# Anannayjain/SNN_Object_DetectionDDP

Measured on NVIDIA B200. Metric: train images/sec, higher is better.
Workload: dtype bf16

## Files before the change

### include/snn_b200.h

```cpp
#ifndef SNN_B200_H
#define SNN_B200_H
#include <stdint.h>
#ifdef __cplusplus
extern "C" {
#endif

const char* snn_last_error(void);
int snn_version(void);
void snn_debug_set(int key, int value);
void snn_set_tile_scheduling(int dynamic);
int snn_conv_plan(int kind, int geom, int NB, int H, int W, int Cin, int Cout, int out_f32, int frames_per_step, int accumulate,
                  int* out20);
void snn_set_deterministic(int on);
int snn_get_deterministic(void);
void snn_set_dependent_launch(int on);
int snn_get_dependent_launch(void);
void snn_tensor_map_cache_stats(unsigned long long* hits, unsigned long long* misses);

enum { SNN_GEOM_3x3_S1 = 0, SNN_GEOM_3x3_S2 = 1, SNN_GEOM_1x1 = 2, SNN_GEOM_T2x2_S2 = 3 };
enum { SNN_ACT_LIF = 0, SNN_ACT_SILU = 1 };

int snn_conv_fprop(int geom, int NB, int H, int W,
                   const void* x0, int C0, long long ld0, const void* x1, int C1, long long ld1,
                   const void* w_bf16, int w_rows, int w_K, int w_coff, int Cout, int w_row_off,
                   const float* bias, void* out, int out_is_f32, long long out_ld, int out_coff,
                   int accumulate, void* stream);
long long snn_conv_stats_groups(int geom, int NB, int H, int W, int frames_per_step, int* groups_per_step);
int snn_conv_fprop_stats(int geom, int NB, int H, int W,
                         const void* x0, int C0, long long ld0, const void* x1, int C1, long long ld1,
                         const void* w_bf16, int w_rows, int w_K, int w_coff, int Cout, int w_row_off,
                         float* out, int frames_per_step, float* partials, void* stream);
int snn_bn_stats_from_partials(const float* partials, double* sums , int T, int C, int groups_per_step,
                               void* stream);
long long snn_bn_finalize_workspace_doubles(int T, int C, int groups_per_step);
int snn_bn_finalize_partials(const float* partials, double* sums, double* workspace, const float* gamma, const float* beta,
                             float* running_mean, float* running_var, long long* num_batches_tracked,
                             float* scale, float* shift, float* mean, float* invstd ,
                             unsigned int* counters, int T, int C, int P, int groups_per_step, float eps, float momentum,
                             void* stream);
int snn_conv_dgrad(int geom, int NB, int H, int W,
                   const void* dy, int Cout, long long ld_dy,
                   const void* w_bf16 , int w_K, int ci_off, int Ci,
                   void* dx, int dx_is_f32, long long dx_ld, int dx_coff, int accumulate, void* stream);
int snn_conv_wgrad(int geom, int NB, int H, int W,
                   const void* x, int Ci, long long ld_x, const void* dy, int Cout, long long ld_dy,
                   float* dw, int w_K, int w_coff, void* stream);
int snn_weight_prep(const float* w, void* w_bf16, void* wt_bf16, int N, int T, int K, void* stream);

long long snn_bn_stats_workspace_floats(int T, int P, int C);
int snn_bn_stats(const float* y, double* sums , float* workspace, int T, int P, int C, void* stream);
int snn_bn_finalize(const double* sums, const float* gamma, const float* beta,
                    float* running_mean, float* running_var,
                    float* scale, float* shift, float* mean, float* invstd ,
                    int T, int C, int P, float eps, float momentum, int training, void* stream);
int snn_bn_act_fwd(int act, const float* y, const float* scale, const float* shift, const float* v_init,
                   void* out_bf16, uint8_t* mask, float* v_final, int T, long long n_per_t, int C,
                   int ss_stride_t, float beta, float theta, void* stream);
int snn_bn_act_bwd(int act, int training, const float* y, const float* scale, const float* shift,
                   const float* mean, const float* invstd, const float* v_init,
                   const void* gs_bf16, const float* gv_final,
                   float* gx, void* dy_bf16, float* gv_init, float* red,
                   int T, int P, int C, int ss_stride_t, float beta, float theta, float alpha, void* stream);
int snn_bn_act_bwd2(int pass, int act, const float* y, const float* scale, const float* shift, const float* mean,
                    const float* invstd, const float* beta_bn, const float* v_init, const void* gs_bf16,
                    const float* gv_final, float* red, void* dy_bf16, float* gv_init, float* dgamma, float* dbeta,
                    int T, int P, int C, float beta, float theta, float alpha, void* stream);
int snn_bn_bwd_dx(const float* red, const float* gamma, const float* gx, const float* y,
                  const float* scale, const float* mean, const float* invstd, float* coef ,
                  float* dgamma, float* dbeta, void* dy_bf16, int T, int P, int C, void* stream);

int snn_lstm_gates_fwd(const float* gates, const float* c_prev, float* c_next, float* h_next,
                       void* h_bf16, long long P, int Ch, void* stream);
int snn_lstm_gates_bwd(const float* gates, const float* c_prev, const float* c_next,
                       const float* dh, const void* dh_bf16, const float* dc_in, void* dgates_bf16, float* dc_prev,
                       long long P, int Ch, void* stream);

int snn_nchw_to_nhwc(const float* in, void* out, int out_is_bf16, int NB, int C, int HW,
                     long long out_ld, int out_coff, void* stream);
int snn_nhwc_to_nchw(const void* in, int in_is_bf16, float* out, int NB, int C, int HW,
                     long long in_ld, int in_coff, void* stream);

int snn_dw3x3_fprop(const void* x_bf16, const float* w, float* y, int NB, int H, int W, int C, void* stream);
int snn_dw3x3_dgrad(const void* dy_bf16, const float* w, void* dx_bf16, int NB, int H, int W, int C, void* stream);
int snn_dw3x3_wgrad(const void* x_bf16, const void* dy_bf16, float* dw, int NB, int H, int W, int C, void* stream);
long long snn_dw3x3_stats_blocks(int frames_per_step, int W, int C);
int snn_dw3x3_fprop_stats(const void* x_bf16, const float* w9c, float* y, int NB, int H, int W, int C, int T, float* partials,
                          void* stream);

int snn_space_to_depth8(const float* frames, void* out_bf16, int B, int T, int H, int W, void* stream);
int snn_space_to_depth8_u8(const unsigned char* frames, void* out_bf16, int B, int T, int H, int W, void* stream);

int snn_bilinear_resize(int backward, const void* src_bf16, void* dst_bf16, int NB, int Hi, int Wi, int Ho, int Wo, int C,
                        void* stream);
int snn_nhwc_pad_crop(const void* src_bf16, void* dst_bf16, int NB, int Hs, int Ws, int Hd, int Wd, int C, void* stream);

int snn_colsum_bf16(const void* dy_bf16, float* acc, long long P, int C, void* stream);

int snn_grad_sumsq(const float* g, long long n, double* acc, int zero_first, void* stream);
int snn_adamw_step(float* p, float* g, float* m, float* v, void* shadow_bf16, long long n,
                   const float* hp, const double* sumsq, float* gnorm_out, int* step_ptr, int n_rows, int zero_grad,
                   void* stream);

int snn_detect_decode(const float* distri, const float* scores, const float* anchors, const float* stride,
                      int B, int A, int nc, int reg_max, int xywh, float* boxes, float* probs, void* stream);

long long snn_nms_workspace_keys(int nc, int A, int multi_label);
int snn_nms(const float* pred, int B, int nc, int A, float conf_thres, float iou_thres, int multi_label, int agnostic,
            int max_det, int max_nms, float max_wh, unsigned long long* keys, long long keys_per_image,
            float* out, int* out_idx, int* counts, void* stream);

int snn_det_match(const float* rows, const int* counts, int B, int max_det, const long long* gt_cls, const float* gt_box,
                  const unsigned char* gt_valid, int M, float img_w, float img_h, const float* iou_thres, int nc,
                  float* rec_conf, int* rec_cls, unsigned short* rec_tp, long long* rec_key, long long capacity,
                  long long* cursor, unsigned int* ticket, long long* n_gt, int* err, void* stream);
int snn_det_metrics_finalize(const long long* keys, const long long* order, const unsigned short* rec_tp, long long n,
                             const long long* n_gt, int nc, const int* err, double* curves, double* out, void* stream);

int snn_detect_loss_fwd(const float* distri, const float* scores, const float* anchors, const float* stride,
                        const float* tbox_px, const float* tscores, const uint8_t* fg, int B, int A, int nc, int reg_max,
                        double* sums, void* stream);
int snn_detect_loss_bwd(const float* distri, const float* scores, const float* anchors, const float* stride,
                        const float* tbox_px, const float* tscores, const uint8_t* fg, int B, int A, int nc, int reg_max,
                        const float* coef, float* g_distri, float* g_scores, void* stream);

long long snn_tal_workspace_bytes(int B, int A, int M);
int snn_detect_assign_loss_fwd(const float* distri, const float* scores, int nl, const int* a_off, const float* anchors,
                               const float* stride, const long long* gt_cls, const float* gt_box, const unsigned char* gt_valid,
                               float img_w, float img_h, int B, int A, int M, int nc, int reg_max, int topk, const float* gains,
                               void* workspace, float* pboxes, float* probs, float* tbox_px, float* tscores, unsigned char* fg,
                               double* sums, unsigned int* counter, float* out6, float* coef3, void* stream);
int snn_tal_assign(const float* probs, const float* pboxes, const float* anchors, const float* stride, const long long* gt_cls,
                   const float* gt_box, const unsigned char* gt_valid, float img_w, float img_h, int B, int A, int M, int nc, int topk,
                   void* workspace, float* tbox_px, float* tscores, unsigned char* fg, void* stream);
int snn_detect_loss_bwd_rows(const float* distri, const float* scores, int nl, const int* a_off, const float* anchors,
                             const float* stride, const float* tbox_px, const float* tscores, const unsigned char* fg, int B, int A,
                             int nc, int reg_max, const float* coef3, const float* gout3, void* g_distri, void* g_scores,
                             int out_is_bf16, void* stream);

#ifdef __cplusplus
}
#endif
#endif
```

### snn_object_detectionddp_b200/_lib.py

```python
import ctypes
import os

import torch

_HERE = os.path.dirname(os.path.abspath(__file__))
LIB_PATH = os.path.join(_HERE, "libsnnb200.so")

GEOM_3x3_S1, GEOM_3x3_S2, GEOM_1x1, GEOM_T2x2_S2 = 0, 1, 2, 3
ACT_LIF, ACT_SILU = 0, 1
GEOM_TAPS = {GEOM_3x3_S1: 9, GEOM_3x3_S2: 9, GEOM_1x1: 1, GEOM_T2x2_S2: 4}

_c = ctypes
_P, _I, _L, _F = _c.c_void_p, _c.c_int, _c.c_longlong, _c.c_float

_SIGNATURES = {
    "snn_conv_fprop": [_I, _I, _I, _I, _P, _I, _L, _P, _I, _L, _P, _I, _I, _I, _I, _I, _P, _P, _I, _L, _I, _I, _P],
    "snn_conv_fprop_stats": [_I, _I, _I, _I, _P, _I, _L, _P, _I, _L, _P, _I, _I, _I, _I, _I, _P, _I, _P, _P],
    "snn_bn_stats_from_partials": [_P, _P, _I, _I, _I, _P],
    "snn_bn_finalize_partials": [_P, _P, _P, _P, _P, _P, _P, _P, _P, _P, _P, _P, _P, _I, _I, _I, _I, _F, _F, _P],
    "snn_conv_dgrad": [_I, _I, _I, _I, _P, _I, _L, _P, _I, _I, _I, _P, _I, _L, _I, _I, _P],
    "snn_conv_wgrad": [_I, _I, _I, _I, _P, _I, _L, _P, _I, _L, _P, _I, _I, _P],
    "snn_weight_prep": [_P, _P, _P, _I, _I, _I, _P],
    "snn_bn_stats": [_P, _P, _P, _I, _I, _I, _P],
    "snn_bn_finalize": [_P, _P, _P, _P, _P, _P, _P, _P, _P, _I, _I, _I, _F, _F, _I, _P],
    "snn_bn_act_fwd": [_I, _P, _P, _P, _P, _P, _P, _P, _I, _L, _I, _I, _F, _F, _P],
    "snn_bn_act_bwd": [_I, _I, _P, _P, _P, _P, _P, _P, _P, _P, _P, _P, _P, _P, _I, _I, _I, _I, _F, _F, _F, _P],
    "snn_bn_act_bwd2": [_I, _I, _P, _P, _P, _P, _P, _P, _P, _P, _P, _P, _P, _P, _P, _P, _I, _I, _I, _F, _F, _F, _P],
    "snn_bn_bwd_dx": [_P, _P, _P, _P, _P, _P, _P, _P, _P, _P, _P, _I, _I, _I, _P],
    "snn_lstm_gates_fwd": [_P, _P, _P, _P, _P, _L, _I, _P],
    "snn_lstm_gates_bwd": [_P, _P, _P, _P, _P, _P, _P, _P, _L, _I, _P],
    "snn_nchw_to_nhwc": [_P, _P, _I, _I, _I, _I, _L, _I, _P],
    "snn_nhwc_to_nchw": [_P, _I, _P, _I, _I, _I, _L, _I, _P],
    "snn_colsum_bf16": [_P, _P, _L, _I, _P],
    "snn_bilinear_resize": [_I, _P, _P, _I, _I, _I, _I, _I, _I, _P],
    "snn_nhwc_pad_crop": [_P, _P, _I, _I, _I, _I, _I, _I, _P],
    "snn_dw3x3_fprop": [_P, _P, _P, _I, _I, _I, _I, _P],
    "snn_dw3x3_fprop_stats": [_P, _P, _P, _I, _I, _I, _I, _I, _P, _P],
    "snn_dw3x3_dgrad": [_P, _P, _P, _I, _I, _I, _I, _P],
    "snn_dw3x3_wgrad": [_P, _P, _P, _I, _I, _I, _I, _P],
    "snn_space_to_depth8": [_P, _P, _I, _I, _I, _I, _P],
    "snn_space_to_depth8_u8": [_P, _P, _I, _I, _I, _I, _P],
    "snn_detect_decode": [_P, _P, _P, _P, _I, _I, _I, _I, _I, _P, _P, _P],
    "snn_detect_loss_fwd": [_P, _P, _P, _P, _P, _P, _P, _I, _I, _I, _I, _P, _P],
    "snn_detect_loss_bwd": [_P, _P, _P, _P, _P, _P, _P, _I, _I, _I, _I, _P, _P, _P, _P],
    "snn_detect_assign_loss_fwd": [_P, _P, _I, _P, _P, _P, _P, _P, _P, _F, _F, _I, _I, _I, _I, _I, _I, _P, _P, _P, _P, _P, _P, _P, _P,
                                   _P, _P, _P, _P],
    "snn_tal_assign": [_P, _P, _P, _P, _P, _P, _P, _F, _F, _I, _I, _I, _I, _I, _P, _P, _P, _P, _P],
    "snn_detect_loss_bwd_rows": [_P, _P, _I, _P, _P, _P, _P, _P, _P, _I, _I, _I, _I, _P, _P, _P, _P, _I, _P],
    "snn_nms": [_P, _I, _I, _I, _F, _F, _I, _I, _I, _I, _F, _P, _L, _P, _P, _P, _P],
    "snn_det_match": [_P, _P, _I, _I, _P, _P, _P, _I, _F, _F, _P, _I, _P, _P, _P, _P, _L, _P, _P, _P, _P, _P],
    "snn_det_metrics_finalize": [_P, _P, _P, _L, _P, _I, _P, _P, _P, _P],
    "snn_grad_sumsq": [_P, _L, _P, _I, _P],
    "snn_adamw_step": [_P, _P, _P, _P, _P, _L, _P, _P, _P, _P, _I, _I, _P],
}

_lib = None
launch_count = 0


class SnnKernelError(RuntimeError):
    pass


def exported_symbols():
    return sorted(list(_SIGNATURES) + ["snn_last_error", "snn_version", "snn_debug_set", "snn_set_tile_scheduling", "snn_set_dependent_launch", "snn_get_dependent_launch", "snn_set_deterministic", "snn_get_deterministic", "snn_conv_plan", "snn_tensor_map_cache_stats", "snn_conv_stats_groups", "snn_bn_stats_workspace_floats", "snn_nms_workspace_keys",
                                             "snn_tal_workspace_bytes", "snn_dw3x3_stats_blocks", "snn_bn_finalize_workspace_doubles"])


def lib():
    global _lib
    if _lib is None:
        if not os.path.isfile(LIB_PATH):
            raise SnnKernelError(
                f"{LIB_PATH} not found: build it with `python -c 'import __graft_entry__ as g; g.build()'` "
                "(nvcc, sm_100a). There is no fallback path.")
        L = ctypes.CDLL(LIB_PATH)
        for name, args in _SIGNATURES.items():
            fn = getattr(L, name)
            fn.argtypes = args
            fn.restype = _I
        L.snn_last_error.restype = ctypes.c_char_p
        L.snn_version.restype = _I
        L.snn_conv_stats_groups.argtypes = [_I, _I, _I, _I, _I, ctypes.POINTER(_I)]
        L.snn_conv_stats_groups.restype = _L
        L.snn_bn_stats_workspace_floats.argtypes = [_I, _I, _I]
        L.snn_bn_stats_workspace_floats.restype = _L
        L.snn_nms_workspace_keys.argtypes = [_I, _I, _I]
        L.snn_nms_workspace_keys.restype = _L
        L.snn_bn_finalize_workspace_doubles.argtypes = [_I, _I, _I]
        L.snn_bn_finalize_workspace_doubles.restype = _L
        L.snn_dw3x3_stats_blocks.argtypes = [_I, _I, _I]
        L.snn_dw3x3_stats_blocks.restype = _L
        L.snn_tal_workspace_bytes.argtypes = [_I, _I, _I]
        L.snn_tal_workspace_bytes.restype = _L
        L.snn_debug_set.argtypes = [_I, _I]
        L.snn_debug_set.restype = None
        if "SNN_WGRAD_STRIP" in os.environ:
            L.snn_debug_set(13, int(os.environ["SNN_WGRAD_STRIP"]))
        if "SNN_WGRAD_ROUNDS" in os.environ:
            L.snn_debug_set(14, int(os.environ["SNN_WGRAD_ROUNDS"]))
        if "SNN_ROW_STRIP" in os.environ:
            L.snn_debug_set(12, int(os.environ["SNN_ROW_STRIP"]))
        L.snn_set_tile_scheduling.argtypes = [_I]
        L.snn_set_tile_scheduling.restype = None
        L.snn_set_dependent_launch.argtypes = [_I]
        L.snn_set_dependent_launch.restype = None
        L.snn_get_dependent_launch.argtypes = []
        L.snn_get_dependent_launch.restype = _I
        L.snn_set_dependent_launch(int(os.environ.get("SNN_DEPENDENT_LAUNCH", "0")))
        L.snn_conv_plan.argtypes = [_I] * 10 + [ctypes.POINTER(_I)]
        L.snn_conv_plan.restype = _I
        L.snn_set_deterministic.argtypes = [_I]
        L.snn_set_deterministic.restype = None
        L.snn_get_deterministic.argtypes = []
        L.snn_get_deterministic.restype = _I
        L.snn_set_deterministic(int(os.environ.get("SNN_DETERMINISTIC", "0")))
        L.snn_tensor_map_cache_stats.argtypes = [ctypes.POINTER(ctypes.c_ulonglong), ctypes.POINTER(ctypes.c_ulonglong)]
        L.snn_tensor_map_cache_stats.restype = None
        _lib = L
    return _lib


def ptr(t):
    if t is None:
        return None
    return t.data_ptr()


_call_dev = None


def stream_ptr():
    return torch.cuda.current_stream(_call_dev).cuda_stream


profile = None
trace = None


def call(name, *args, work=None):
    global launch_count
    dev = _call_dev
    if profile is not None:
        e0 = torch.cuda.Event(enable_timing=True)
        e0.record(torch.cuda.current_stream(dev))
    fn = getattr(lib(), name)
    if dev is not None and dev.index is not None and dev.index != torch.cuda.current_device():
        with torch.cuda.device(dev):
            rc = fn(*args)
    else:
        rc = fn(*args)
    if rc != 0:
        raise SnnKernelError(f"{name} failed (rc={rc}): {lib().snn_last_error().decode()}")
    launch_count += 1
    if trace is not None:
        trace.append((name, work))
    if profile is not None:
        e1 = torch.cuda.Event(enable_timing=True)
        e1.record(torch.cuda.current_stream(dev))
        profile.append((name, work, e0, e1))


def require_cuda(*tensors):
    global _call_dev
    dev = None
    for t in tensors:
        if t is None:
            continue
        if not t.is_cuda:
            raise SnnKernelError("snn_object_detectionddp_b200 kernels run on CUDA tensors only (no CPU fallback)")
        if dev is None:
            dev = t.device
        elif t.device != dev:
            raise SnnKernelError(f"tensors of one kernel call live on different devices ({dev} vs {t.device})")
    _call_dev = dev
    return dev
```

### snn_object_detectionddp_b200/csrc/api.cu

```cuda
#include <stdarg.h>

#include <atomic>
#include <mutex>
#include <stdio.h>

#include "../../include/snn_b200.h"
#include "common.cuh"

namespace snn {

static thread_local char g_err[1024] = "";

void set_error(const char* fmt, ...) {
    va_list ap;
    va_start(ap, fmt);
    vsnprintf(g_err, sizeof(g_err), fmt, ap);
    va_end(ap);
}
int check_cuda(cudaError_t e, const char* what) {
    if (e == cudaSuccess) return 0;
    set_error("CUDA error %d (%s) at %s", (int)e, cudaGetErrorString(e), what);
    return 1;
}
int current_device() {
    int dev = 0;
    return cudaGetDevice(&dev) == cudaSuccess ? dev : -1;
}
int num_sms() {
    static std::atomic<int> cache[64];
    const int dev = current_device();
    if (dev >= 0 && dev < 64) {
        const int c = cache[dev].load(std::memory_order_relaxed);
        if (c > 0) return c;
    }
    int n = 0;
    if (dev < 0 || cudaDeviceGetAttribute(&n, cudaDevAttrMultiProcessorCount, dev) != cudaSuccess || n <= 0) n = 148;
    if (dev >= 0 && dev < 64) cache[dev].store(n, std::memory_order_relaxed);
    return n;
}

static std::atomic<int> g_pdl{0};
bool pdl_enabled() { return g_pdl.load(std::memory_order_relaxed) != 0; }
void set_pdl(int on) { g_pdl.store(on ? 1 : 0, std::memory_order_relaxed); }

static std::atomic<int> g_det{0};
bool deterministic() { return g_det.load(std::memory_order_relaxed) != 0; }
void set_deterministic(int on) { g_det.store(on ? 1 : 0, std::memory_order_relaxed); }

static void* g_det_ws[64];
static size_t g_det_ws_bytes[64];
static std::mutex g_det_mutex;
void* det_scratch(size_t bytes, cudaStream_t st) {
    const int dev = current_device();
    if (dev < 0 || dev >= 64) { set_error("deterministic mode: bad CUDA device %d", dev); return nullptr; }
    std::lock_guard<std::mutex> g(g_det_mutex);
    if (g_det_ws_bytes[dev] >= bytes) return g_det_ws[dev];
    cudaStreamCaptureStatus cs = cudaStreamCaptureStatusNone;
    if (cudaStreamIsCapturing(st, &cs) != cudaSuccess || cs != cudaStreamCaptureStatusNone) {
        set_error("deterministic mode: the scratch buffer (%zu bytes) must be allocated outside CUDA-graph capture: run the step once eagerly first", bytes);
        return nullptr;
    }
    size_t want = bytes < ((size_t)64 << 20) ? ((size_t)64 << 20) : bytes;
    void* q = nullptr;
    if (cudaDeviceSynchronize() != cudaSuccess || cudaMalloc(&q, want) != cudaSuccess) {
        set_error("deterministic mode: cudaMalloc(%zu) failed", want);
        return nullptr;
    }
    if (g_det_ws[dev]) cudaFree(g_det_ws[dev]);
    g_det_ws[dev] = q; g_det_ws_bytes[dev] = want;
    return q;
}

void debug_set(int k, int v);
void set_dynamic_tiles(int on);
void tmap_cache_stats(unsigned long long*, unsigned long long*);
int conv_plan(int, int, int, int, int, int, int, int, int, int, int*);
int conv_fprop(int, int, int, int, const void*, int, long long, const void*, int, long long, const void*, int, int, int, int,
               int, const float*, void*, int, long long, int, int, cudaStream_t, float*, int);
long long conv_stats_groups(int, int, int, int, int, int*);
long long nms_workspace_keys(int, int, int);
int launch_nms(const float*, int, int, int, float, float, int, int, int, int, float, unsigned long long*, long long, float*, int*,
               int*, cudaStream_t);
int launch_bn_stats_from_partials(const float*, double*, int, int, int, cudaStream_t);
int launch_bn_finalize_partials(const float*, double*, double*, const float*, const float*, float*, float*, long long*, float*, float*,
                                float*, float*, unsigned int*, int, int, int, int, float, float, cudaStream_t);
long long bn_finalize_workspace_doubles(int, int, int);
int conv_dgrad(int, int, int, int, const void*, int, long long, const void*, int, int, int, void*, int, long long, int, int,
               cudaStream_t);
int conv_wgrad(int, int, int, int, const void*, int, long long, const void*, int, long long, float*, int, int, cudaStream_t);
int launch_weight_prep(const float*, __nv_bfloat16*, __nv_bfloat16*, int, int, int, cudaStream_t);
int launch_bn_stats(const float*, double*, float*, int, int, int, cudaStream_t);
long long bn_stats_workspace_floats(int, int, int);
int launch_bn_finalize(const double*, const float*, const float*, float*, float*, float*, float*, float*, float*, int, int, int,
                       float, float, int, cudaStream_t);
int launch_bn_act_fwd(int, const float*, const float*, const float*, const float*, __nv_bfloat16*, uint8_t*, float*, int,
                      long long, int, int, float, float, cudaStream_t);
int launch_bn_act_bwd(int, int, const float*, const float*, const float*, const float*, const float*, const float*,
                      const __nv_bfloat16*, const float*, float*, __nv_bfloat16*, float*, float*, int, int, int, int, float,
                      float, float, cudaStream_t);
int launch_bn_act_bwd2(int, int, const float*, const float*, const float*, const float*, const float*, const float*,
                       const float*, const __nv_bfloat16*, const float*, float*, __nv_bfloat16*, float*, float*, float*, int, int,
                       int, float, float, float, cudaStream_t);
int launch_bn_bwd_dx(const float*, const float*, const float*, const float*, const float*, const float*, const float*, float*,
                     float*, float*, __nv_bfloat16*, int, int, int, cudaStream_t);
int launch_lstm_gates_fwd(const float*, const float*, float*, float*, __nv_bfloat16*, long long, int, cudaStream_t);
int launch_lstm_gates_bwd(const float*, const float*, const float*, const float*, const __nv_bfloat16*, const float*, __nv_bfloat16*,
                          float*, long long, int, cudaStream_t);
int launch_nchw_to_nhwc(const float*, void*, int, int, int, int, long long, int, cudaStream_t);
int launch_nhwc_to_nchw(const void*, int, float*, int, int, int, long long, int, cudaStream_t);
int launch_sumsq(const float*, long long, double*, int, cudaStream_t);
int launch_colsum_bf16(const __nv_bfloat16*, float*, long long, int, cudaStream_t);
int launch_dw3x3_fwd(const __nv_bfloat16*, const float*, float*, int, int, int, int, float*, int, cudaStream_t);
long long dw3x3_stats_blocks(int, int, int);
int launch_dw3x3_dgrad(const __nv_bfloat16*, const float*, __nv_bfloat16*, int, int, int, int, cudaStream_t);
int launch_dw3x3_wgrad(const __nv_bfloat16*, const __nv_bfloat16*, float*, int, int, int, int, cudaStream_t);
int launch_s2d8(const float*, __nv_bfloat16*, int, int, int, int, cudaStream_t);
int launch_s2d8_u8(const uint8_t*, __nv_bfloat16*, int, int, int, int, cudaStream_t);
int launch_adamw(float*, float*, float*, float*, __nv_bfloat16*, long long, const float*, const double*, float*,
                 int*, int, int, cudaStream_t);
int launch_bilinear(int, const __nv_bfloat16*, __nv_bfloat16*, int, int, int, int, int, int, cudaStream_t);
int launch_pad_crop(const __nv_bfloat16*, __nv_bfloat16*, int, int, int, int, int, int, cudaStream_t);
int launch_detect_decode(const float*, const float*, const float*, const float*, int, int, int, int, int, float*, float*, int,
                         const int*, cudaStream_t);
int launch_detect_loss_fwd(const float*, const float*, const float*, const float*, const float*, const float*, const uint8_t*,
                           int, int, int, int, double*, int, const int*, const float*, int, const float*, unsigned int*, float*,
                           float*, cudaStream_t);
int launch_detect_loss_bwd(const float*, const float*, const float*, const float*, const float*, const float*, const uint8_t*,
                           int, int, int, int, const float*, const float*, void*, void*, int, int, const int*, cudaStream_t);
long long tal_workspace_bytes(int, int, int);
int launch_tal_assign(const float*, const float*, const float*, const float*, const long long*, const float*, const uint8_t*, float,
                      float, int, int, int, int, int, void*, float*, float*, uint8_t*, float**, int*, cudaStream_t);

int launch_det_match(const float*, const int*, int, int, const long long*, const float*, const unsigned char*, int, float, float,
                     const float*, int, float*, int*, unsigned short*, long long*, long long, long long*, unsigned int*,
                     long long*, int*, cudaStream_t);
int launch_det_metrics_finalize(const long long*, const long long*, const unsigned short*, long long, const long long*, int,
                                const int*, double*, double*, cudaStream_t);

}

using namespace snn;
#define ST ((cudaStream_t)stream)

extern "C" {

const char* snn_last_error(void) { return g_err; }
int snn_version(void) { return 100; }
void snn_debug_set(int key, int value) { debug_set(key, value); }
void snn_set_tile_scheduling(int dynamic) { set_dynamic_tiles(dynamic); }
int snn_conv_plan(int kind, int geom, int NB, int H, int W, int Cin, int Cout, int out_f32, int frames_per_step, int accumulate, int* out20) {
    return conv_plan(kind, geom, NB, H, W, Cin, Cout, out_f32, frames_per_step, accumulate, out20);
}
void snn_set_deterministic(int on) { set_deterministic(on); }
int snn_get_deterministic(void) { return deterministic() ? 1 : 0; }
void snn_set_dependent_launch(int on) { set_pdl(on); }
int snn_get_dependent_launch(void) { return pdl_enabled() ? 1 : 0; }
void snn_tensor_map_cache_stats(unsigned long long* hits, unsigned long long* misses) { tmap_cache_stats(hits, misses); }

int snn_conv_fprop(int geom, int NB, int H, int W, const void* x0, int C0, long long ld0, const void* x1, int C1,
                   long long ld1, const void* w, int w_rows, int w_K, int w_coff, int Cout, int w_row_off,
                   const float* bias, void* out, int out_is_f32, long long out_ld, int out_coff, int accumulate,
                   void* stream) {
    return conv_fprop(geom, NB, H, W, x0, C0, ld0, x1, C1, ld1, w, w_rows, w_K, w_coff, Cout, w_row_off, bias, out,
                      out_is_f32, out_ld, out_coff, accumulate, ST, nullptr, 0);
}
long long snn_conv_stats_groups(int geom, int NB, int H, int W, int frames_per_step, int* groups_per_step) {
    return conv_stats_groups(geom, NB, H, W, frames_per_step, groups_per_step);
}
int snn_conv_fprop_stats(int geom, int NB, int H, int W, const void* x0, int C0, long long ld0, const void* x1, int C1,
                         long long ld1, const void* w, int w_rows, int w_K, int w_coff, int Cout, int w_row_off, float* out,
                         int frames_per_step, float* partials, void* stream) {
    return conv_fprop(geom, NB, H, W, x0, C0, ld0, x1, C1, ld1, w, w_rows, w_K, w_coff, Cout, w_row_off, nullptr, out, 1,
                      Cout, 0, 0, ST, partials, frames_per_step);
}
long long snn_nms_workspace_keys(int nc, int A, int multi_label) { return nms_workspace_keys(nc, A, multi_label && nc > 1); }
int snn_nms(const float* pred, int B, int nc, int A, float conf_thres, float iou_thres, int multi_label, int agnostic,
            int max_det, int max_nms, float max_wh, unsigned long long* keys, long long keys_per_image, float* out,
            int* out_idx, int* counts, void* stream) {
    return launch_nms(pred, B, nc, A, conf_thres, iou_thres, multi_label, agnostic, max_det, max_nms, max_wh, keys,
                      keys_per_image, out, out_idx, counts, ST);
}
int snn_det_match(const float* rows, const int* counts, int B, int max_det, const long long* gt_cls, const float* gt_box,
                  const unsigned char* gt_valid, int M, float img_w, float img_h, const float* iou_thres, int nc,
                  float* rec_conf, int* rec_cls, unsigned short* rec_tp, long long* rec_key, long long capacity,
                  long long* cursor, unsigned int* ticket, long long* n_gt, int* err, void* stream) {
    return launch_det_match(rows, counts, B, max_det, gt_cls, gt_box, gt_valid, M, img_w, img_h, iou_thres, nc, rec_conf, rec_cls,
                            rec_tp, rec_key, capacity, cursor, ticket, n_gt, err, ST);
}
int snn_det_metrics_finalize(const long long* keys, const long long* order, const unsigned short* rec_tp, long long n,
                             const long long* n_gt, int nc, const int* err, double* curves, double* out, void* stream) {
    return launch_det_metrics_finalize(keys, order, rec_tp, n, n_gt, nc, err, curves, out, ST);
}
long long snn_bn_finalize_workspace_doubles(int T, int C, int groups_per_step) { return bn_finalize_workspace_doubles(T, C, groups_per_step); }
int snn_bn_finalize_partials(const float* partials, double* sums, double* workspace, const float* gamma, const float* beta,
                             float* running_mean, float* running_var, long long* num_batches_tracked, float* scale, float* shift,
                             float* mean, float* invstd, unsigned int* counters, int T, int C, int P, int groups_per_step, float eps,
                             float momentum, void* stream) {
    return launch_bn_finalize_partials(partials, sums, workspace, gamma, beta, running_mean, running_var, num_batches_tracked, scale,
                                       shift, mean, invstd, counters, T, C, P, groups_per_step, eps, momentum, ST);
}
int snn_bn_stats_from_partials(const float* partials, double* sums, int T, int C, int groups_per_step, void* stream) {
    return launch_bn_stats_from_partials(partials, sums, T, C, groups_per_step, ST);
}
int snn_conv_dgrad(int geom, int NB, int H, int W, const void* dy, int Cout, long long ld_dy, const void* wt, int wt_rows,
                   int ci_off, int Ci, void* dx, int dx_is_f32, long long dx_ld, int dx_coff, int accumulate, void* stream) {
    return conv_dgrad(geom, NB, H, W, dy, Cout, ld_dy, wt, wt_rows, ci_off, Ci, dx, dx_is_f32, dx_ld, dx_coff, accumulate, ST);
}
int snn_conv_wgrad(int geom, int NB, int H, int W, const void* x, int Ci, long long ld_x, const void* dy, int Cout,
                   long long ld_dy, float* dw, int w_K, int w_coff, void* stream) {
    return conv_wgrad(geom, NB, H, W, x, Ci, ld_x, dy, Cout, ld_dy, dw, w_K, w_coff, ST);
}
int snn_weight_prep(const float* w, void* wf, void* wt, int N, int T, int K, void* stream) {
    return launch_weight_prep(w, (__nv_bfloat16*)wf, (__nv_bfloat16*)wt, N, T, K, ST);
}
int snn_bn_stats(const float* y, double* sums, float* workspace, int T, int P, int C, void* stream) {
    return launch_bn_stats(y, sums, workspace, T, P, C, ST);
}
long long snn_bn_stats_workspace_floats(int T, int P, int C) { return bn_stats_workspace_floats(T, P, C); }
int snn_bn_finalize(const double* sums, const float* gamma, const float* beta, float* rm, float* rv, float* scale,
                    float* shift, float* mean, float* invstd, int T, int C, int P, float eps, float momentum, int training,
                    void* stream) {
    return launch_bn_finalize(sums, gamma, beta, rm, rv, scale, shift, mean, invstd, T, C, P, eps, momentum, training, ST);
}
int snn_bn_act_fwd(int act, const float* y, const float* scale, const float* shift, const float* v_init, void* out,
                   uint8_t* mask, float* v_final, int T, long long n_per_t, int C, int ss_stride_t, float beta, float theta,
                   void* stream) {
    return launch_bn_act_fwd(act, y, scale, shift, v_init, (__nv_bfloat16*)out, mask, v_final, T, n_per_t, C, ss_stride_t,
                             beta, theta, ST);
}
int snn_bn_act_bwd(int act, int training, const float* y, const float* scale, const float* shift, const float* mean,
                   const float* invstd, const float* v_init, const void* gs, const float* gv_final, float* gx, void* dy,
                   float* gv_init, float* red, int T, int P, int C, int ss_stride_t, float beta, float theta, float alpha,
                   void* stream) {
    return launch_bn_act_bwd(act, training, y, scale, shift, mean, invstd, v_init, (const __nv_bfloat16*)gs, gv_final, gx,
                             (__nv_bfloat16*)dy, gv_init, red, T, P, C, ss_stride_t, beta, theta, alpha, ST);
}
int snn_bn_act_bwd2(int pass, int act, const float* y, const float* scale, const float* shift, const float* mean,
                    const float* invstd, const float* beta_bn, const float* v_init, const void* gs, const float* gv_final,
                    float* red, void* dy, float* gv_init, float* dgamma, float* dbeta, int T, int P, int C, float beta,
                    float theta, float alpha, void* stream) {
    return launch_bn_act_bwd2(pass, act, y, scale, shift, mean, invstd, beta_bn, v_init, (const __nv_bfloat16*)gs, gv_final,
                              red, (__nv_bfloat16*)dy, gv_init, dgamma, dbeta, T, P, C, beta, theta, alpha, ST);
}
int snn_bn_bwd_dx(const float* red, const float* gamma, const float* gx, const float* y, const float* scale,
                  const float* mean, const float* invstd, float* coef, float* dgamma, float* dbeta, void* dy, int T, int P,
                  int C, void* stream) {
    return launch_bn_bwd_dx(red, gamma, gx, y, scale, mean, invstd, coef, dgamma, dbeta, (__nv_bfloat16*)dy, T, P, C, ST);
}
int snn_lstm_gates_fwd(const float* gates, const float* c_prev, float* c_next, float* h_next, void* h_bf16, long long P,
                       int Ch, void* stream) {
    return launch_lstm_gates_fwd(gates, c_prev, c_next, h_next, (__nv_bfloat16*)h_bf16, P, Ch, ST);
}
int snn_lstm_gates_bwd(const float* gates, const float* c_prev, const float* c_next, const float* dh, const void* dh_bf16,
                       const float* dc_in, void* dgates, float* dc_prev, long long P, int Ch, void* stream) {
    return launch_lstm_gates_bwd(gates, c_prev, c_next, dh, (const __nv_bfloat16*)dh_bf16, dc_in, (__nv_bfloat16*)dgates, dc_prev, P, Ch, ST);
}
int snn_nchw_to_nhwc(const float* in, void* out, int out_is_bf16, int NB, int C, int HW, long long out_ld, int out_coff,
                     void* stream) {
    return launch_nchw_to_nhwc(in, out, out_is_bf16, NB, C, HW, out_ld, out_coff, ST);
}
int snn_nhwc_to_nchw(const void* in, int in_is_bf16, float* out, int NB, int C, int HW, long long in_ld, int in_coff,
                     void* stream) {
    return launch_nhwc_to_nchw(in, in_is_bf16, out, NB, C, HW, in_ld, in_coff, ST);
}
int snn_dw3x3_fprop(const void* x, const float* w, float* y, int NB, int H, int W, int C, void* stream) {
    return launch_dw3x3_fwd((const __nv_bfloat16*)x, w, y, NB, H, W, C, nullptr, 0, ST);
}
long long snn_dw3x3_stats_blocks(int frames_per_step, int W, int C) { return dw3x3_stats_blocks(frames_per_step, W, C); }
int snn_dw3x3_fprop_stats(const void* x, const float* w, float* y, int NB, int H, int W, int C, int T, float* partials, void* stream) {
    return launch_dw3x3_fwd((const __nv_bfloat16*)x, w, y, NB, H, W, C, partials, T, ST);
}
int snn_dw3x3_dgrad(const void* dy, const float* w, void* dx, int NB, int H, int W, int C, void* stream) {
    return launch_dw3x3_dgrad((const __nv_bfloat16*)dy, w, (__nv_bfloat16*)dx, NB, H, W, C, ST);
}
int snn_dw3x3_wgrad(const void* x, const void* dy, float* dw, int NB, int H, int W, int C, void* stream) {
    return launch_dw3x3_wgrad((const __nv_bfloat16*)x, (const __nv_bfloat16*)dy, dw, NB, H, W, C, ST);
}
int snn_space_to_depth8(const float* frames, void* out, int B, int T, int H, int W, void* stream) {
    return launch_s2d8(frames, (__nv_bfloat16*)out, B, T, H, W, ST);
}
int snn_space_to_depth8_u8(const unsigned char* frames, void* out, int B, int T, int H, int W, void* stream) {
    return launch_s2d8_u8(frames, (__nv_bfloat16*)out, B, T, H, W, ST);
}
int snn_bilinear_resize(int backward, const void* src, void* dst, int NB, int Hi, int Wi, int Ho, int Wo, int C, void* stream) {
    return launch_bilinear(backward, (const __nv_bfloat16*)src, (__nv_bfloat16*)dst, NB, Hi, Wi, Ho, Wo, C, ST);
}
int snn_nhwc_pad_crop(const void* src, void* dst, int NB, int Hs, int Ws, int Hd, int Wd, int C, void* stream) {
    return launch_pad_crop((const __nv_bfloat16*)src, (__nv_bfloat16*)dst, NB, Hs, Ws, Hd, Wd, C, ST);
}
int snn_colsum_bf16(const void* dy, float* acc, long long P, int C, void* stream) {
    return launch_colsum_bf16((const __nv_bfloat16*)dy, acc, P, C, ST);
}
int snn_grad_sumsq(const float* g, long long n, double* acc, int zero_first, void* stream) {
    return launch_sumsq(g, n, acc, zero_first, ST);
}
int snn_adamw_step(float* p, float* g, float* m, float* v, void* shadow, long long n, const float* hp,
                   const double* sumsq, float* gnorm_out, int* step_ptr, int n_rows, int zero_grad, void* stream) {
    return launch_adamw(p, g, m, v, (__nv_bfloat16*)shadow, n, hp, sumsq, gnorm_out, step_ptr, n_rows, zero_grad, ST);
}
int snn_detect_decode(const float* distri, const float* scores, const float* anchors, const float* stride, int B, int A,
                      int nc, int reg_max, int xywh, float* boxes, float* probs, void* stream) {
    return launch_detect_decode(distri, scores, anchors, stride, B, A, nc, reg_max, xywh, boxes, probs, 0, nullptr, ST);
}
int snn_detect_loss_fwd(const float* distri, const float* scores, const float* anchors, const float* stride,
                        const float* tbox_px, const float* tscores, const uint8_t* fg, int B, int A, int nc, int reg_max,
                        double* sums, void* stream) {
    return launch_detect_loss_fwd(distri, scores, anchors, stride, tbox_px, tscores, fg, B, A, nc, reg_max, sums, 0, nullptr, nullptr, 0,
                                  nullptr, nullptr, nullptr, nullptr, ST);
}
int snn_detect_loss_bwd(const float* distri, const float* scores, const float* anchors, const float* stride,
                        const float* tbox_px, const float* tscores, const uint8_t* fg, int B, int A, int nc, int reg_max,
                        const float* coef, float* g_distri, float* g_scores, void* stream) {
    return launch_detect_loss_bwd(distri, scores, anchors, stride, tbox_px, tscores, fg, B, A, nc, reg_max, coef, nullptr, g_distri,
                                  g_scores, 0, 0, nullptr, ST);
}
long long snn_tal_workspace_bytes(int B, int A, int M) { return tal_workspace_bytes(B, A, M); }
int snn_detect_assign_loss_fwd(const float* distri, const float* scores, int nl, const int* a_off, const float* anchors,
                               const float* stride, const long long* gt_cls, const float* gt_box, const unsigned char* gt_valid,
                               float img_w, float img_h, int B, int A, int M, int nc, int reg_max, int topk, const float* gains,
                               void* workspace, float* pboxes, float* probs, float* tbox_px, float* tscores, unsigned char* fg,
                               double* sums, unsigned int* counter, float* out6, float* coef3, void* stream) {
    int rc = launch_detect_decode(distri, scores, anchors, stride, B, A, nc, reg_max, 0, pboxes, probs, nl, a_off, ST);
    if (rc) return rc;
    float* tss_part = nullptr;
    int n_parts = 0;
    rc = launch_tal_assign(probs, pboxes, anchors, stride, gt_cls, gt_box, gt_valid, img_w, img_h, B, A, M, nc, topk, workspace, tbox_px,
                           tscores, fg, &tss_part, &n_parts, ST);
    if (rc) return rc;
    return launch_detect_loss_fwd(distri, scores, anchors, stride, tbox_px, tscores, fg, B, A, nc, reg_max, sums, nl, a_off, tss_part,
                                  n_parts, gains, counter, out6, coef3, ST);
}
int snn_tal_assign(const float* probs, const float* pboxes, const float* anchors, const float* stride, const long long* gt_cls,
                   const float* gt_box, const unsigned char* gt_valid, float img_w, float img_h, int B, int A, int M, int nc, int topk,
                   void* workspace, float* tbox_px, float* tscores, unsigned char* fg, void* stream) {
    return launch_tal_assign(probs, pboxes, anchors, stride, gt_cls, gt_box, gt_valid, img_w, img_h, B, A, M, nc, topk, workspace, tbox_px,
                             tscores, fg, nullptr, nullptr, ST);
}
int snn_detect_loss_bwd_rows(const float* distri, const float* scores, int nl, const int* a_off, const float* anchors,
                             const float* stride, const float* tbox_px, const float* tscores, const unsigned char* fg, int B, int A,
                             int nc, int reg_max, const float* coef3, const float* gout3, void* g_distri, void* g_scores,
                             int out_is_bf16, void* stream) {
    return launch_detect_loss_bwd(distri, scores, anchors, stride, tbox_px, tscores, fg, B, A, nc, reg_max, coef3, gout3, g_distri,
                                  g_scores, out_is_bf16, nl, a_off, ST);
}

}
```

### snn_object_detectionddp_b200/csrc/gemm_tc.cu

```cuda
#include <atomic>
#include <mutex>
#include <unordered_map>

#include "common.cuh"

namespace snn {

struct Seg {
    int src, dc, dw, dhp, dh;
    int wtap, wc0, nchunk;
};
struct Phase {
    int nseg, oph, opw, pad;
    Seg seg[18];
};
struct ConvGemmParams {
    int NB, Hd, Wd;
    int bn, bh, bw;
    int tiles_w, tiles_h, tiles_n;
    int BN;
    int n_blocks;
    int n_store;
    int wn_off;
    int stages, stage_bytes;
    void* out;
    const float* bias;
    int out_f32, accumulate;
    int Ho, Wo, os;
    long long out_ld;
    int out_coff;
    int nphase;
    int b_mn;
    int b_boxes;
    float* stats;
    int tma_out;
    int cps, chunk_bytes;
    int nbuf;
    int epi_groups;
    unsigned int* sched;
    int ksplit;
    int dbg;
    int ntap, a_bytes, a_tap_off, b_bytes, tap_wstep;
    int hnw;
    Phase phase[4];
};

struct WTap {
    int g_dc, g_dw, g_dhp, g_dh;
    int x_dc, x_dw, x_dhp, x_dh;
    int wtap, pad0, pad1, pad2;
};
struct WgradParams {
    int NB, Hd, Wd;
    int bn, bh, bw;
    int tiles_w, tiles_h, tiles_n, total_tiles;
    int ksplit, tiles_per_split;
    int m_items;
    int NT;
    int n_ci_tiles;
    int Cout, Ci;
    float* dw;
    long long dw_ld;
    int wK, w_coff;
    int stages, stage_bytes;
    int lbo_bytes, sbo_bytes;
    int ntaps;
    int strip, x_box_bytes, x_tap_off;
    int hnw;
    unsigned int* sched;
    WTap taps[9];
};

constexpr int kMaxStages = 8;
constexpr int kTmemCols = 256;

constexpr int kAccCols = 256;

template <bool PAIR>
__global__ void __launch_bounds__(320, 1)
conv_gemm_kernel(const __grid_constant__ CUtensorMap tmA0, const __grid_constant__ CUtensorMap tmA1,
                 const __grid_constant__ CUtensorMap tmB, const __grid_constant__ CUtensorMap tmO,
                 const __grid_constant__ ConvGemmParams p) {
    extern __shared__ uint8_t smem_raw[];
    __shared__ __align__(8) uint64_t full_bar[kMaxStages];
    __shared__ __align__(8) uint64_t empty_bar[kMaxStages];
    __shared__ __align__(8) uint64_t tmem_full_bar[2];
    __shared__ __align__(8) uint64_t tmem_empty_bar[2];
    __shared__ SchedRing ring;
    __shared__ uint32_t tmem_base_s;

    pdl_launch_dependents();
    const int warp = __shfl_sync(0xffffffffu, (int)(threadIdx.x >> 5), 0), lane = threadIdx.x & 31;
    const uint32_t sbase = (smem_u32(smem_raw) + 1023u) & ~1023u;
    const int stages = p.stages;
    const uint32_t stage_bytes = (uint32_t)p.stage_bytes;
    const uint32_t rank = PAIR ? cluster_ctarank() : 0u;
    const int worker = PAIR ? (int)(blockIdx.x >> 1) : (int)blockIdx.x;
    const int nworkers = PAIR ? (int)(gridDim.x >> 1) : (int)gridDim.x;
    const int m_tiles = p.tiles_w * p.tiles_h * p.tiles_n;
    const int m_work = PAIR ? (m_tiles + 1) >> 1 : m_tiles;
    const int total_tiles = m_work * p.n_blocks * p.nphase * p.ksplit;
    const int bn_cta = PAIR ? p.BN >> 1 : p.BN;

    if (warp == 0) {
        if (lane == 0) {
            tma_prefetch_desc(&tmA0);
            tma_prefetch_desc(&tmA1);
            tma_prefetch_desc(&tmB);
            if (p.tma_out) tma_prefetch_desc(&tmO);
        }
        __syncwarp();
        if (PAIR) tmem_alloc_pair<2 * kAccCols>(smem_u32(&tmem_base_s));
        else tmem_alloc<2 * kAccCols>(smem_u32(&tmem_base_s));
    } else if (warp == 1 && lane == 0) {
        for (int s = 0; s < stages; ++s) {
            mbar_init(smem_u32(&full_bar[s]), 1);
            mbar_init(smem_u32(&empty_bar[s]), 1);
        }
        for (int a = 0; a < 2; ++a) {
            mbar_init(smem_u32(&tmem_full_bar[a]), 1);
            mbar_init(smem_u32(&tmem_empty_bar[a]), (PAIR ? 8u : 4u) * (uint32_t)p.epi_groups);
        }
        sched_init(ring, (PAIR ? 2u : 1u) * (1u + 4u * (uint32_t)p.epi_groups));
        mbar_fence_init();
    }
    tc_fence_before();
    if (PAIR) cluster_sync_all(); else __syncthreads();
    tc_fence_after();
    const uint32_t tmem_base = tmem_base_s;
    pdl_wait();

    if (warp == 0) {
        const bool lead = elect_one();
        int s = 0;
        uint32_t par = 0;
        uint32_t a_s = sbase;
        const bool dyn = p.sched != nullptr;
        int tile = worker, nxt1 = -1, pend = 0, pub = 0;
        if (dyn && rank == 0) {
            if (tile >= total_tiles) tile = -1;
            sched_publish<PAIR>(ring, pub++, tile, lead);
            if (tile < 0) pub = -1;
            if (pub > 0) {
                if (lane == 0) pend = (int)atomicAdd(p.sched, 1u) + nworkers;
                nxt1 = __shfl_sync(0xffffffffu, pend, 0);
                if (nxt1 >= total_tiles) nxt1 = -1;
                sched_publish<PAIR>(ring, pub++, nxt1, lead);
                if (nxt1 < 0) pub = -1;
                else if (lane == 0) pend = (int)atomicAdd(p.sched, 1u) + nworkers;
            }
        }
        for (int it = 0;; ++it) {
            if (!dyn) {
                tile = worker + it * nworkers;
                if (tile >= total_tiles) break;
            } else if (rank == 0) {
                if (tile < 0) break;
            } else {
                tile = sched_next<PAIR>(ring, it, lane);
                if (tile < 0) break;
            }
            const int mt = (tile % m_work) * (PAIR ? 2 : 1) + (int)rank, rest = tile / m_work;
            const int ncol0 = p.wn_off + (rest % p.n_blocks) * p.BN + (int)rank * bn_cta;
            const int pk = rest / p.n_blocks;
            const Phase& ph = p.phase[pk % p.nphase];
            const int tw = mt % p.tiles_w, th = (mt / p.tiles_w) % p.tiles_h, tn = mt / (p.tiles_w * p.tiles_h);
            const int w0 = tw * p.bw, h0 = th * p.bh, n0 = tn * p.bn;
            const int spp = ph.nseg / p.ksplit, sg0 = (pk / p.nphase) * spp;
            for (int sg = sg0; sg < sg0 + spp; ++sg) {
                const Seg g = ph.seg[sg];
                const CUtensorMap* tmA = g.src ? &tmA1 : &tmA0;
                const int cw = w0 + g.dw, chh = h0 + g.dh;
                int ca = g.dc, cb = g.wc0;
                for (int kc = 0; kc < g.nchunk; kc += p.cps) {
                    const int nsub = min(p.cps, g.nchunk - kc);
                    mbar_wait(smem_u32(&empty_bar[s]), par ^ 1u);
                    if (lead) {
                        const uint32_t fb = smem_u32(&full_bar[s]);
#ifdef SNN_TIMING_KNOBS
                        if (p.dbg & 1) {
                            if (rank == 0) mbar_arrive(fb);
                        } else
#endif
                        if (!PAIR) {
                            mbar_expect_tx(fb, (uint32_t)(nsub * p.chunk_bytes));
                            for (int j = 0; j < nsub; ++j) {
                                const uint32_t c_s = a_s + (uint32_t)(j * p.chunk_bytes);
                                tma_load_5d(c_s, tmA, fb, ca + 64 * j, cw, g.dhp, p.hnw ? n0 : chh, p.hnw ? chh : n0);
                                for (int tp = 0; tp < p.ntap; ++tp) {
                                    const uint32_t b_s = c_s + (uint32_t)(p.a_bytes + tp * p.b_bytes);
                                    const int wt = g.wtap + tp * p.tap_wstep;
                                    if (!p.b_mn) {
                                        tma_load_3d(b_s, &tmB, fb, cb + 64 * j, wt, ncol0);
                                    } else {
                                        for (int nb = 0; nb < p.b_boxes; ++nb)
                                            tma_load_3d(b_s + (uint32_t)nb * 8192u, &tmB, fb, ncol0 + nb * 64, wt, cb + 64 * j);
                                    }
                                }
                            }
                        } else {
                            if (rank == 0) mbar_expect_tx(fb, 2u * (uint32_t)(nsub * p.chunk_bytes));
                            for (int j = 0; j < nsub; ++j) {
                                const uint32_t c_s = a_s + (uint32_t)(j * p.chunk_bytes);
                                tma_load_5d_pair(c_s, tmA, fb, ca + 64 * j, cw, g.dhp, p.hnw ? n0 : chh, p.hnw ? chh : n0);
                                for (int tp = 0; tp < p.ntap; ++tp) {
                                    const uint32_t b_s = c_s + (uint32_t)(p.a_bytes + tp * p.b_bytes);
                                    const int wt = g.wtap + tp * p.tap_wstep;
                                    if (!p.b_mn) {
                                        tma_load_3d_pair(b_s, &tmB, fb, cb + 64 * j, wt, ncol0);
                                    } else {
                                        for (int nb = 0; nb < p.b_boxes; ++nb)
                                            tma_load_3d_pair(b_s + (uint32_t)nb * 8192u, &tmB, fb, ncol0 + nb * 64, wt, cb + 64 * j);
                                    }
                                }
                            }
                        }
                    }
                    ca += 64 * p.cps; cb += 64 * p.cps;
                    a_s += stage_bytes;
                    if (++s == stages) { s = 0; par ^= 1u; a_s = sbase; }
                }
            }
            if (dyn && rank == 0) {
                tile = nxt1;
                if (pub > 0) {
                    nxt1 = __shfl_sync(0xffffffffu, pend, 0);
                    if (nxt1 >= total_tiles) nxt1 = -1;
                    sched_publish<PAIR>(ring, pub++, nxt1, lead);
                    if (nxt1 < 0) pub = -1;
                    else if (lane == 0) pend = (int)atomicAdd(p.sched, 1u) + nworkers;
                } else {
                    nxt1 = -1;
                }
            }
        }
    } else if (warp == 1) {
        if (rank == 0) {
            const bool lead = elect_one();
            const uint32_t idesc = umma_idesc_bf16(PAIR ? 256 : 128, p.BN, 0, p.b_mn);
            const uint32_t desc_hi = (1024u >> 4) | (1u << 14) | (2u << 29);
            const uint32_t a_lo_c = (16u >> 4) << 16;
            const uint32_t b_lo_c = (p.b_mn ? (8192u >> 4) : (16u >> 4)) << 16;
            const uint32_t b_kstep = p.b_mn ? (2048u >> 4) : (32u >> 4);
#ifdef SNN_TIMING_KNOBS
            const uint32_t dbg_nomma = (uint32_t)(p.dbg & 2);
#else
            constexpr uint32_t dbg_nomma = 0u;
#endif
            int s = 0, lt = 0;
            uint32_t par = 0;
            uint32_t a_s = sbase;
            const bool dyn = p.sched != nullptr;
            for (;; ++lt) {
                const int tile = dyn ? sched_next<PAIR>(ring, lt, lane) : (worker + lt * nworkers < total_tiles ? worker + lt * nworkers : -1);
                if (tile < 0) break;
                const int pk = (tile / m_work) / p.n_blocks;
                const Phase& ph = p.phase[pk % p.nphase];
                const int spp = ph.nseg / p.ksplit, sg0 = (pk / p.nphase) * spp;
                const int acc = lt & 1;
                mbar_wait(smem_u32(&tmem_empty_bar[acc]), (uint32_t)(((lt >> 1) & 1) ^ 1));
                tc_fence_after();
                const uint32_t tacc = tmem_base + (uint32_t)(acc * kAccCols);
                uint32_t first = 1u;
                for (int sg = sg0; sg < sg0 + spp; ++sg) {
                    const int nchunk = ph.seg[sg].nchunk;
                    const bool last_seg = sg == sg0 + spp - 1;
                    for (int kc = 0; kc < nchunk; kc += p.cps) {
                        const int nsub = min(p.cps, nchunk - kc);
                        mbar_wait(smem_u32(&full_bar[s]), par);
                        tc_fence_after();
                        if (lead) {
                            if (!dbg_nomma) {
                                for (int j = 0; j < nsub; ++j) {
                                    const uint32_t c_s = a_s + (uint32_t)(j * p.chunk_bytes);
                                    for (int tp = 0; tp < p.ntap; ++tp) {
                                        const uint32_t a_lo = a_lo_c | (((c_s + (uint32_t)(tp * p.a_tap_off)) & 0x3FFFFu) >> 4);
                                        const uint32_t b_lo = b_lo_c | (((c_s + (uint32_t)(p.a_bytes + tp * p.b_bytes)) & 0x3FFFFu) >> 4);
#pragma unroll
                                        for (int k = 0; k < 4; ++k) {
                                            const uint64_t adesc = ((uint64_t)desc_hi << 32) | (uint64_t)(a_lo + 2u * k);
                                            const uint64_t bdesc = ((uint64_t)desc_hi << 32) | (uint64_t)(b_lo + b_kstep * k);
                                            const uint32_t accf = (k | j | tp) ? 1u : (first ^ 1u);
                                            if (PAIR) umma_bf16_pair(tacc, adesc, bdesc, idesc, accf);
                                            else umma_bf16(tacc, adesc, bdesc, idesc, accf);
                                        }
                                    }
                                }
                            }
                            if (PAIR) umma_commit_pair(smem_u32(&empty_bar[s])); else umma_commit(smem_u32(&empty_bar[s]));
                            if (last_seg && kc + p.cps >= nchunk) {
                                if (PAIR) umma_commit_pair(smem_u32(&tmem_full_bar[acc])); else umma_commit(smem_u32(&tmem_full_bar[acc]));
                            }
                        }
                        first = 0u;
                        a_s += stage_bytes;
                        if (++s == stages) { s = 0; par ^= 1u; a_s = sbase; }
                    }
                }
            }
        }
    } else {
        const int q = warp & 3;
        const int grp = warp >= 6 ? 1 : 0, ngrp = p.epi_groups;
        const int row = q * 32 + lane;
        const int wl = row % p.bw;
        const int hl = p.hnw ? row / (p.bw * p.bn) : (row / p.bw) % p.bh, nl = p.hnw ? (row / p.bw) % p.bn : row / (p.bw * p.bh);
        int lt = 0;
        uint32_t gcc = 0;
        const bool dyn = p.sched != nullptr;
        for (;; ++lt) {
            const int tile = dyn ? sched_next<PAIR>(ring, lt, lane) : (worker + lt * nworkers < total_tiles ? worker + lt * nworkers : -1);
            if (tile < 0) break;
            const int mt = (tile % m_work) * (PAIR ? 2 : 1) + (int)rank, rest = tile / m_work;
            const int ncol0 = (rest % p.n_blocks) * p.BN;
            const Phase& ph = p.phase[(rest / p.n_blocks) % p.nphase];
            const int tw = mt % p.tiles_w, th = (mt / p.tiles_w) % p.tiles_h, tn = mt / (p.tiles_w * p.tiles_h);
            const int n = tn * p.bn + nl, hd = th * p.bh + hl, wd = tw * p.bw + wl;
            const bool valid = (n < p.NB) && (hd < p.Hd) && (wd < p.Wd);
            const long long pix = ((long long)n * p.Ho + (hd * p.os + ph.oph)) * p.Wo + (wd * p.os + ph.opw);
            const int acc = lt & 1;
            mbar_wait(smem_u32(&tmem_full_bar[acc]), (uint32_t)((lt >> 1) & 1));
            tc_fence_after();
            const uint32_t trow = tmem_base + (uint32_t)(acc * kAccCols) + ((uint32_t)(q * 32) << 16);
            if (p.tma_out) {
                const int CH = p.out_f32 ? 32 : 64;
                const int chs = p.out_f32 ? 5 : 6;
                const int row0 = q * 32;
                const int bw_ = p.bw, bh_ = p.bh;
                const int cw = tw * bw_ + row0 % bw_;
                const int chh = th * bh_ + (p.hnw ? row0 / (bw_ * p.bn) : (row0 / bw_) % bh_);
                const int cn = tn * p.bn + (p.hnw ? (row0 / bw_) % p.bn : row0 / (bw_ * bh_));
                const int c3 = p.hnw ? cn : chh, c4 = p.hnw ? chh : cn;
                const int cbase = (p.os == 2 ? ph.opw * (int)p.out_ld : 0);
                const int cph = (p.os == 2 ? ph.oph : 0);
                const uint32_t stg0 = sbase + (uint32_t)stages * stage_bytes + (uint32_t)((grp * 4 + q) * p.nbuf) * 4096u;
                const int nch = (min(p.BN, p.n_store - ncol0) + CH - 1) >> chs;
                const bool has_bias = p.bias != nullptr;
                for (int cc = grp; cc < nch; cc += ngrp, ++gcc) {
                    const uint32_t buf = stg0 + (gcc & (uint32_t)(p.nbuf - 1)) * 4096u;
                    uint32_t r[32];
                    if (p.out_f32) {
                        tmem_ld16(trow + (uint32_t)(cc * 32), r);
                        tmem_ld16(trow + (uint32_t)(cc * 32 + 16), r + 16);
                        tmem_ld_wait();
                        if (has_bias) {
                            const int c0 = ncol0 + cc * 32;
#pragma unroll
                            for (int j4 = 0; j4 < 8; ++j4) {
                                float4 bv = make_float4(0.f, 0.f, 0.f, 0.f);
                                if (c0 + 4 * j4 < p.n_store) bv = __ldg(reinterpret_cast<const float4*>(p.bias + c0) + j4);
                                r[4 * j4 + 0] = __float_as_uint(__uint_as_float(r[4 * j4 + 0]) + bv.x);
                                r[4 * j4 + 1] = __float_as_uint(__uint_as_float(r[4 * j4 + 1]) + bv.y);
                                r[4 * j4 + 2] = __float_as_uint(__uint_as_float(r[4 * j4 + 2]) + bv.z);
                                r[4 * j4 + 3] = __float_as_uint(__uint_as_float(r[4 * j4 + 3]) + bv.w);
                            }
                        }
                    } else {
#pragma unroll
                        for (int hh = 0; hh < 2; ++hh) {
                            uint32_t t32[32];
                            tmem_ld16(trow + (uint32_t)(cc * 64 + hh * 32), t32);
                            tmem_ld16(trow + (uint32_t)(cc * 64 + hh * 32 + 16), t32 + 16);
                            tmem_ld_wait();
                            if (has_bias) {
                                const int c0 = ncol0 + cc * 64 + hh * 32;
#pragma unroll
                                for (int j4 = 0; j4 < 8; ++j4) {
                                    float4 bv = make_float4(0.f, 0.f, 0.f, 0.f);
                                    if (c0 + 4 * j4 < p.n_store) bv = __ldg(reinterpret_cast<const float4*>(p.bias + c0) + j4);
                                    r[hh * 16 + 2 * j4] = pack_bf16x2(__uint_as_float(t32[4 * j4]) + bv.x, __uint_as_float(t32[4 * j4 + 1]) + bv.y);
                                    r[hh * 16 + 2 * j4 + 1] = pack_bf16x2(__uint_as_float(t32[4 * j4 + 2]) + bv.z, __uint_as_float(t32[4 * j4 + 3]) + bv.w);
                                }
                            } else {
#pragma unroll
                                for (int j = 0; j < 16; ++j)
                                    r[hh * 16 + j] = pack_bf16x2(__uint_as_float(t32[2 * j]), __uint_as_float(t32[2 * j + 1]));
                            }
                        }
                    }
                    if (gcc >= (uint32_t)p.nbuf) {
                        if (lane == 0) { if (p.nbuf == 4) bulk_wait_group_read<3>(); else bulk_wait_group_read<1>(); }
                        __syncwarp();
                    }
                    if (p.stats && !valid) {
#pragma unroll
                        for (int j = 0; j < 32; ++j) r[j] = 0u;
                    }
                    const uint32_t rowaddr = buf + (uint32_t)lane * 128u;
#pragma unroll
                    for (int c = 0; c < 8; ++c)
                        st_shared_v4(rowaddr + (uint32_t)((c ^ (lane & 7)) << 4), r[4 * c], r[4 * c + 1], r[4 * c + 2], r[4 * c + 3]);
                    fence_proxy_async_smem();
                    __syncwarp();
                    if (p.stats && mt < m_tiles) {
                        float sm = 0.f, sq = 0.f;
                        const uint32_t cadr = buf + (uint32_t)((lane & 3) << 2);
#pragma unroll 8
                        for (int rr = 0; rr < 32; ++rr) {
                            float v;
                            asm volatile("ld.shared.f32 %0, [%1];" : "=f"(v) : "r"(cadr + (uint32_t)rr * 128u + (uint32_t)((((lane >> 2) ^ (rr & 7))) << 4)));
                            sm += v;
                            sq = fmaf(v, v, sq);
                        }
                        const int col = ncol0 + cc * 32 + lane;
                        if (col < p.n_store) {
                            float* dst = p.stats + ((size_t)(mt * 4 + q) * 2) * (size_t)p.n_store + col;
                            dst[0] = sm;
                            dst[p.n_store] = sq;
                        }
                    }
                    if (lane == 0) {
                        if (p.accumulate) tma_reduce_add_5d(&tmO, buf, cbase + ncol0 + cc * CH, cw, cph, c3, c4);
                        else tma_store_5d(&tmO, buf, cbase + ncol0 + cc * CH, cw, cph, c3, c4);
                        bulk_commit_group();
                    }
                }
                tc_fence_before();
                __syncwarp();
                if (lane == 0) {
                    if (PAIR) mbar_arrive_cluster(smem_u32(&tmem_empty_bar[acc]) & kPeerBitMask);
                    else mbar_arrive(smem_u32(&tmem_empty_bar[acc]));
                }
                continue;
            }
            const int nchunks = p.BN >> 4;
            for (int ch = grp; ch < nchunks; ch += ngrp) {
                uint32_t r[16];
                tmem_ld16(trow + (uint32_t)(ch * 16), r);
                tmem_ld_wait();
                const int col = ncol0 + ch * 16;
                if (!valid || col >= p.n_store) continue;
                const int nv = min(16, p.n_store - col);
                float v[16];
#pragma unroll
                for (int j = 0; j < 16; ++j) v[j] = __uint_as_float(r[j]);
                if (p.bias) {
#pragma unroll
                    for (int j = 0; j < 16; ++j)
                        if (j < nv) v[j] += __ldg(p.bias + col + j);
                }
                if (p.out_f32) {
                    float4* o = reinterpret_cast<float4*>(reinterpret_cast<float*>(p.out) + pix * p.out_ld + p.out_coff + col);
#pragma unroll
                    for (int j = 0; j < 4; ++j) {
                        if (j * 4 < nv) {
                            float4 t = make_float4(v[4 * j], v[4 * j + 1], v[4 * j + 2], v[4 * j + 3]);
                            if (p.accumulate) {
                                const float4 old = o[j];
                                t.x += old.x; t.y += old.y; t.z += old.z; t.w += old.w;
                            }
                            o[j] = t;
                        }
                    }
                } else {
                    __nv_bfloat16* ob = reinterpret_cast<__nv_bfloat16*>(p.out) + pix * p.out_ld + p.out_coff + col;
                    uint4* o = reinterpret_cast<uint4*>(ob);
#pragma unroll
                    for (int j = 0; j < 2; ++j) {
                        if (j * 8 < nv) {
                            if (p.accumulate) {
                                const uint4 old = o[j];
                                v[8 * j + 0] += bf16_lo(old.x); v[8 * j + 1] += bf16_hi(old.x);
                                v[8 * j + 2] += bf16_lo(old.y); v[8 * j + 3] += bf16_hi(old.y);
                                v[8 * j + 4] += bf16_lo(old.z); v[8 * j + 5] += bf16_hi(old.z);
                                v[8 * j + 6] += bf16_lo(old.w); v[8 * j + 7] += bf16_hi(old.w);
                            }
                            uint4 t;
                            t.x = pack_bf16x2(v[8 * j + 0], v[8 * j + 1]); t.y = pack_bf16x2(v[8 * j + 2], v[8 * j + 3]);
                            t.z = pack_bf16x2(v[8 * j + 4], v[8 * j + 5]); t.w = pack_bf16x2(v[8 * j + 6], v[8 * j + 7]);
                            o[j] = t;
                        }
                    }
                }
            }
            tc_fence_before();
            __syncwarp();
            if (lane == 0) {
                if (PAIR) mbar_arrive_cluster(smem_u32(&tmem_empty_bar[acc]) & kPeerBitMask);
                else mbar_arrive(smem_u32(&tmem_empty_bar[acc]));
            }
        }
    }
    if (p.tma_out && warp >= 2 && lane == 0) bulk_wait_group<0>();
    __syncwarp();
    tc_fence_before();
    if (PAIR) {
        cluster_sync_all();
        if (warp == 0) { __syncwarp(); tmem_dealloc_pair<2 * kAccCols>(tmem_base); }
    } else {
        __syncthreads();
        if (warp == 0) tmem_dealloc<2 * kAccCols>(tmem_base);
    }
    if (p.sched != nullptr && rank == 0 && threadIdx.x == 0) sched_finish(p.sched, nworkers);
}

template <bool PAIR>
__global__ void __launch_bounds__(192, 1)
wgrad_gemm_kernel(const __grid_constant__ CUtensorMap tmG, const __grid_constant__ CUtensorMap tmX,
                  const __grid_constant__ CUtensorMap tmW, const __grid_constant__ WgradParams p) {
    extern __shared__ uint8_t smem_raw[];
    __shared__ __align__(8) uint64_t full_bar[kMaxStages];
    __shared__ __align__(8) uint64_t empty_bar[kMaxStages];
    __shared__ __align__(8) uint64_t tmem_full_bar[2];
    __shared__ __align__(8) uint64_t tmem_empty_bar[2];
    __shared__ SchedRing ring;
    __shared__ uint32_t tmem_base_s;

    pdl_launch_dependents();
    const int warp = __shfl_sync(0xffffffffu, (int)(threadIdx.x >> 5), 0), lane = threadIdx.x & 31;
    const uint32_t sbase = (smem_u32(smem_raw) + 1023u) & ~1023u;
    const int stages = p.stages;
    const uint32_t stage_bytes = (uint32_t)p.stage_bytes;
    constexpr uint32_t kBox = 64 * 128;
    const uint32_t rank = PAIR ? cluster_ctarank() : 0u;
    const int worker = PAIR ? (int)(blockIdx.x >> 1) : (int)blockIdx.x;
    const int nworkers = PAIR ? (int)(gridDim.x >> 1) : (int)gridDim.x;
    const int ny = p.n_ci_tiles * p.ntaps;
    const int total_items = p.m_items * ny * p.ksplit;
    const int nxb = (PAIR ? p.NT >> 1 : p.NT) >> 6;
    const uint32_t xbb = p.strip ? (uint32_t)p.x_box_bytes : kBox;
    const int ntp = p.strip ? 3 : 1;
    const int tiles_hw = p.tiles_w * p.tiles_h;

    if (warp == 0) {
        if (lane == 0) {
            tma_prefetch_desc(&tmG);
            tma_prefetch_desc(&tmX);
            tma_prefetch_desc(&tmW);
        }
        __syncwarp();
        if (PAIR) tmem_alloc_pair<2 * kTmemCols>(smem_u32(&tmem_base_s)); else tmem_alloc<2 * kTmemCols>(smem_u32(&tmem_base_s));
    } else if (warp == 1 && lane == 0) {
        for (int s = 0; s < stages; ++s) {
            mbar_init(smem_u32(&full_bar[s]), 1);
            mbar_init(smem_u32(&empty_bar[s]), 1);
        }
        for (int a = 0; a < 2; ++a) {
            mbar_init(smem_u32(&tmem_full_bar[a]), 1);
            mbar_init(smem_u32(&tmem_empty_bar[a]), PAIR ? 8 : 4);
        }
        sched_init(ring, PAIR ? 10u : 5u);
        mbar_fence_init();
    }
    tc_fence_before();
    if (PAIR) cluster_sync_all(); else __syncthreads();
    tc_fence_after();
    const uint32_t tmem_base = tmem_base_s;
    pdl_wait();

    if (warp == 0) {
        const bool lead = elect_one();
        int s = 0;
        uint32_t par = 0;
        uint32_t g_s = sbase;
        const bool dyn = p.sched != nullptr;
        int item = worker, nxt1 = -1, pend = 0, pub = 0;
        if (dyn && rank == 0) {
            if (item >= total_items) item = -1;
            sched_publish<PAIR>(ring, pub++, item, lead);
            if (item < 0) pub = -1;
            if (pub > 0) {
                if (lane == 0) pend = (int)atomicAdd(p.sched, 1u) + nworkers;
                nxt1 = __shfl_sync(0xffffffffu, pend, 0);
                if (nxt1 >= total_items) nxt1 = -1;
                sched_publish<PAIR>(ring, pub++, nxt1, lead);
                if (nxt1 < 0) pub = -1;
                else if (lane == 0) pend = (int)atomicAdd(p.sched, 1u) + nworkers;
            }
        }
        for (int seq = 0;; ++seq) {
            if (!dyn) {
                item = worker + seq * nworkers;
                if (item >= total_items) break;
            } else if (rank == 0) {
                if (item < 0) break;
            } else {
                item = sched_next<PAIR>(ring, seq, lane);
                if (item < 0) break;
            }
            const int mi = item % p.m_items, y = (item / p.m_items) % ny, z = item / (p.m_items * ny);
            const int co0 = PAIR ? mi * 256 + (int)rank * 128 : mi * 128;
            const WTap tp = p.taps[y / p.n_ci_tiles];
            const int ci0 = (y % p.n_ci_tiles) * p.NT + (PAIR ? (int)rank * (p.NT >> 1) : 0);
            const int t_begin = z * p.tiles_per_split;
            const int total = min(p.total_tiles, t_begin + p.tiles_per_split) - t_begin;
            int tw = t_begin % p.tiles_w, th = (t_begin / p.tiles_w) % p.tiles_h, tn = t_begin / tiles_hw;
            const int gc0 = tp.g_dc + co0, xc0 = tp.x_dc + ci0;
            for (int it = 0; it < total; ++it) {
                const int w0 = tw * p.bw, h0 = th * p.bh, n0 = tn * p.bn;
                mbar_wait(smem_u32(&empty_bar[s]), par ^ 1u);
                if (lead) {
                    const uint32_t fb = smem_u32(&full_bar[s]);
                    const uint32_t x_s = g_s + 2 * kBox;
                    if (!PAIR) {
                        mbar_expect_tx(fb, stage_bytes);
                        tma_load_5d(g_s, &tmG, fb, gc0, w0 + tp.g_dw, tp.g_dhp, p.hnw ? n0 : h0 + tp.g_dh, p.hnw ? h0 + tp.g_dh : n0);
                        tma_load_5d(g_s + kBox, &tmG, fb, gc0 + 64, w0 + tp.g_dw, tp.g_dhp, p.hnw ? n0 : h0 + tp.g_dh, p.hnw ? h0 + tp.g_dh : n0);
                        for (int b = 0; b < nxb; ++b)
                            tma_load_5d(x_s + b * xbb, &tmX, fb, xc0 + b * 64, w0 + tp.x_dw, tp.x_dhp, p.hnw ? n0 : h0 + tp.x_dh, p.hnw ? h0 + tp.x_dh : n0);
                    } else {
                        if (rank == 0) mbar_expect_tx(fb, 2u * stage_bytes);
                        tma_load_5d_pair(g_s, &tmG, fb, gc0, w0 + tp.g_dw, tp.g_dhp, p.hnw ? n0 : h0 + tp.g_dh, p.hnw ? h0 + tp.g_dh : n0);
                        tma_load_5d_pair(g_s + kBox, &tmG, fb, gc0 + 64, w0 + tp.g_dw, tp.g_dhp, p.hnw ? n0 : h0 + tp.g_dh, p.hnw ? h0 + tp.g_dh : n0);
                        for (int b = 0; b < nxb; ++b)
                            tma_load_5d_pair(x_s + b * xbb, &tmX, fb, xc0 + b * 64, w0 + tp.x_dw, tp.x_dhp, p.hnw ? n0 : h0 + tp.x_dh, p.hnw ? h0 + tp.x_dh : n0);
                    }
                }
                g_s += stage_bytes;
                if (++s == stages) { s = 0; par ^= 1u; g_s = sbase; }
                if (++tw == p.tiles_w) { tw = 0; if (++th == p.tiles_h) { th = 0; ++tn; } }
            }
            if (dyn && rank == 0) {
                item = nxt1;
                if (pub > 0) {
                    nxt1 = __shfl_sync(0xffffffffu, pend, 0);
                    if (nxt1 >= total_items) nxt1 = -1;
                    sched_publish<PAIR>(ring, pub++, nxt1, lead);
                    if (nxt1 < 0) pub = -1;
                    else if (lane == 0) pend = (int)atomicAdd(p.sched, 1u) + nworkers;
                } else {
                    nxt1 = -1;
                }
            }
        }
    } else if (warp == 1) {
        if (rank == 0) {
            const bool lead = elect_one();
            const uint32_t idesc = umma_idesc_bf16(PAIR ? 256 : 128, p.NT, 1, 1);
            const uint32_t desc_hi = ((uint32_t)p.sbo_bytes >> 4) | (1u << 14) | (2u << 29);
            const uint32_t lo_c = (((uint32_t)p.lbo_bytes >> 4) & 0x3FFFu) << 16;
            const uint32_t lo_cb = p.strip ? ((((uint32_t)p.x_box_bytes >> 4) & 0x3FFFu) << 16) : lo_c;
            int s = 0, li = 0;
            uint32_t par = 0;
            uint32_t g_s = sbase;
            const bool dyn = p.sched != nullptr;
            for (;; ++li) {
                const int item = dyn ? sched_next<PAIR>(ring, li, lane) : (worker + li * nworkers < total_items ? worker + li * nworkers : -1);
                if (item < 0) break;
                const int t_begin = (item / (p.m_items * ny)) * p.tiles_per_split;
                const int total = min(p.total_tiles, t_begin + p.tiles_per_split) - t_begin;
                const int acc = p.strip ? 0 : (li & 1);
                mbar_wait(smem_u32(&tmem_empty_bar[acc]), (uint32_t)(((p.strip ? li : (li >> 1)) & 1) ^ 1));
                tc_fence_after();
                const uint32_t tacc = tmem_base + (uint32_t)(acc * kTmemCols);
                for (int it = 0; it < total; ++it) {
                    mbar_wait(smem_u32(&full_bar[s]), par);
                    tc_fence_after();
                    if (lead) {
                        const uint32_t a_lo = lo_c | ((g_s & 0x3FFFFu) >> 4);
                        for (int t3 = 0; t3 < ntp; ++t3) {
                            const uint32_t b_lo = lo_cb | (((g_s + 2 * kBox + (uint32_t)(t3 * p.x_tap_off)) & 0x3FFFFu) >> 4);
                            const uint32_t tcol = tacc + (uint32_t)(t3 * p.NT);
#pragma unroll
                            for (int k = 0; k < 4; ++k) {
                                const uint64_t adesc = ((uint64_t)desc_hi << 32) | (uint64_t)(a_lo + (2048u >> 4) * k);
                                const uint64_t bdesc = ((uint64_t)desc_hi << 32) | (uint64_t)(b_lo + (2048u >> 4) * k);
                                if (PAIR) umma_bf16_pair(tcol, adesc, bdesc, idesc, k ? 1u : (uint32_t)(it != 0));
                                else umma_bf16(tcol, adesc, bdesc, idesc, k ? 1u : (uint32_t)(it != 0));
                            }
                        }
                        if (PAIR) umma_commit_pair(smem_u32(&empty_bar[s])); else umma_commit(smem_u32(&empty_bar[s]));
                        if (it == total - 1) {
                            if (PAIR) umma_commit_pair(smem_u32(&tmem_full_bar[acc])); else umma_commit(smem_u32(&tmem_full_bar[acc]));
                        }
                    }
                    g_s += stage_bytes;
                    if (++s == stages) { s = 0; par ^= 1u; g_s = sbase; }
                }
            }
        }
    } else {
        const int q = warp & 3;
        const uint32_t stg0 = sbase + (uint32_t)stages * stage_bytes + (uint32_t)q * 8192u;
        uint32_t gcc = 0;
        int li = 0;
        const bool dyn = p.sched != nullptr;
        for (;; ++li) {
            const int item = dyn ? sched_next<PAIR>(ring, li, lane) : (worker + li * nworkers < total_items ? worker + li * nworkers : -1);
            if (item < 0) break;
            const int mi = item % p.m_items, y = (item / p.m_items) % ny;
            const int co0 = (PAIR ? mi * 256 + (int)rank * 128 : mi * 128) + q * 32;
            const int wtap = p.taps[y / p.n_ci_tiles].wtap;
            const int ci0 = (y % p.n_ci_tiles) * p.NT;
            const int acc = p.strip ? 0 : (li & 1);
            mbar_wait(smem_u32(&tmem_full_bar[acc]), (uint32_t)((p.strip ? li : (li >> 1)) & 1));
            tc_fence_after();
            const uint32_t trow = tmem_base + (uint32_t)(acc * kTmemCols) + ((uint32_t)(q * 32) << 16);
            const int nch = (min(p.NT, p.Ci - ci0) + 31) >> 5;
            for (int c3 = 0; c3 < nch * ntp; ++c3, ++gcc) {
                const int t3 = c3 / nch, cc = c3 - t3 * nch;
                const uint32_t buf = stg0 + (gcc & 1u) * 4096u;
                uint32_t r[32];
                tmem_ld16(trow + (uint32_t)(t3 * p.NT + cc * 32), r);
                tmem_ld16(trow + (uint32_t)(t3 * p.NT + cc * 32 + 16), r + 16);
                tmem_ld_wait();
                if (gcc >= 2) {
                    if (lane == 0) bulk_wait_group_read<1>();
                    __syncwarp();
                }
                const uint32_t rowaddr = buf + (uint32_t)lane * 128u;
#pragma unroll
                for (int c = 0; c < 8; ++c)
                    st_shared_v4(rowaddr + (uint32_t)((c ^ (lane & 7)) << 4), r[4 * c], r[4 * c + 1], r[4 * c + 2], r[4 * c + 3]);
                fence_proxy_async_smem();
                __syncwarp();
                if (lane == 0 && co0 < p.Cout) {
                    tma_reduce_add_3d(&tmW, buf, p.w_coff + ci0 + cc * 32, wtap + 3 * t3, co0);
                    bulk_commit_group();
                }
            }
            tc_fence_before();
            __syncwarp();
            if (lane == 0) {
                if (PAIR) mbar_arrive_cluster(smem_u32(&tmem_empty_bar[acc]) & kPeerBitMask);
                else mbar_arrive(smem_u32(&tmem_empty_bar[acc]));
            }
        }
        if (lane == 0) bulk_wait_group<0>();
    }
    __syncwarp();
    tc_fence_before();
    if (PAIR) {
        cluster_sync_all();
        if (warp == 0) { __syncwarp(); tmem_dealloc_pair<2 * kTmemCols>(tmem_base); }
    } else {
        __syncthreads();
        if (warp == 0) tmem_dealloc<2 * kTmemCols>(tmem_base);
    }
    if (p.sched != nullptr && rank == 0 && threadIdx.x == 0) sched_finish(p.sched, nworkers);
}

static std::once_flag g_encode_once;

struct TmapKey {
    unsigned long long ptr, dims[5], strides[4];
    unsigned int box[5], dtype, rank, swizzle, l2, dev;
    bool operator==(const TmapKey& o) const { return memcmp(this, &o, sizeof(TmapKey)) == 0; }
};
struct TmapKeyHash {
    size_t operator()(const TmapKey& k) const {
        const unsigned long long* w = reinterpret_cast<const unsigned long long*>(&k);
        unsigned long long h = 1469598103934665603ull;
        for (size_t i = 0; i < sizeof(TmapKey) / 8; ++i) { h ^= w[i]; h *= 1099511628211ull; }
        return (size_t)h;
    }
};
static_assert(sizeof(TmapKey) % 8 == 0, "TmapKey is hashed as 64-bit words");
constexpr size_t kTmapCacheMax = 16384;
static std::unordered_map<TmapKey, CUtensorMap, TmapKeyHash> g_tmap_cache;
static std::mutex g_tmap_mutex;
static std::atomic<unsigned long long> g_tmap_hits{0}, g_tmap_misses{0};
void tmap_cache_stats(unsigned long long* hits, unsigned long long* misses) {
    *hits = g_tmap_hits.load(); *misses = g_tmap_misses.load();
}

typedef CUresult (*EncodeTiledFn)(CUtensorMap*, CUtensorMapDataType, cuuint32_t, void*, const cuuint64_t*,
                                  const cuuint64_t*, const cuuint32_t*, const cuuint32_t*, CUtensorMapInterleave,
                                  CUtensorMapSwizzle, CUtensorMapL2promotion, CUtensorMapFloatOOBfill);
static EncodeTiledFn g_encode_raw = nullptr;

static CUresult g_encode(CUtensorMap* m, CUtensorMapDataType dt, cuuint32_t rank, void* ptr, const cuuint64_t* dims, const cuuint64_t* strides,
                         const cuuint32_t* box, const cuuint32_t* es, CUtensorMapInterleave il, CUtensorMapSwizzle sw, CUtensorMapL2promotion l2,
                         CUtensorMapFloatOOBfill oob) {
    TmapKey k;
    memset(&k, 0, sizeof(k));
    k.ptr = (unsigned long long)(uintptr_t)ptr; k.dtype = (unsigned)dt; k.rank = rank; k.swizzle = (unsigned)sw; k.l2 = (unsigned)l2;
    k.dev = (unsigned)current_device();
    for (cuuint32_t i = 0; i < rank; ++i) { k.dims[i] = dims[i]; k.box[i] = box[i]; }
    for (cuuint32_t i = 0; i + 1 < rank; ++i) k.strides[i] = strides[i];
    {
        std::lock_guard<std::mutex> g(g_tmap_mutex);
        auto it = g_tmap_cache.find(k);
        if (it != g_tmap_cache.end()) { *m = it->second; g_tmap_hits.fetch_add(1, std::memory_order_relaxed); return CUDA_SUCCESS; }
    }
    const CUresult r = g_encode_raw(m, dt, rank, ptr, dims, strides, box, es, il, sw, l2, oob);
    if (r == CUDA_SUCCESS) {
        std::lock_guard<std::mutex> g(g_tmap_mutex);
        if (g_tmap_cache.size() >= kTmapCacheMax) g_tmap_cache.clear();
        g_tmap_cache.emplace(k, *m);
        g_tmap_misses.fetch_add(1, std::memory_order_relaxed);
    }
    return r;
}

struct PlanSink { bool active = false; int v[24]; };
static thread_local PlanSink t_plan;

static int get_encode() {
    std::call_once(g_encode_once, [] {
        void* fn = nullptr;
        cudaDriverEntryPointQueryResult qres;
        cudaError_t e = cudaGetDriverEntryPoint("cuTensorMapEncodeTiled", &fn, cudaEnableDefault, &qres);
        if (e == cudaSuccess && qres == cudaDriverEntryPointSuccess) g_encode_raw = (EncodeTiledFn)fn;
    });
    SNN_REQUIRE(g_encode_raw != nullptr, "cuTensorMapEncodeTiled not available from the CUDA driver");
    return 0;
}

static int make_act_map(CUtensorMap* m, const void* ptr, int NB, int H, int W, int C, long long ld, int phase_view,
                        int box_n, int box_h, int box_w, int hnw = 0) {
    if (t_plan.active) return 0;
    if (get_encode()) return 2;
    SNN_REQUIRE(((uintptr_t)ptr & 15) == 0, "activation pointer must be 16-byte aligned");
    SNN_REQUIRE(ld % 8 == 0 && C % 8 == 0, "activation channels/stride must be multiples of 8 (C=%d ld=%lld)", C, ld);
    cuuint64_t dims[5], strides[4];
    cuuint32_t box[5] = {64, (cuuint32_t)box_w, 1, (cuuint32_t)box_h, (cuuint32_t)box_n}, es[5] = {1, 1, 1, 1, 1};
    if (!phase_view && hnw) {
        dims[0] = C; dims[1] = W; dims[2] = 1; dims[3] = NB; dims[4] = H;
        strides[0] = ld * 2; strides[1] = (cuuint64_t)W * ld * 2; strides[2] = (cuuint64_t)H * W * ld * 2;
        strides[3] = (cuuint64_t)W * ld * 2;
        box[3] = (cuuint32_t)box_n; box[4] = (cuuint32_t)box_h;
    } else if (!phase_view) {
        dims[0] = C; dims[1] = W; dims[2] = 1; dims[3] = H; dims[4] = NB;
        strides[0] = ld * 2; strides[1] = (cuuint64_t)W * ld * 2; strides[2] = (cuuint64_t)W * ld * 2;
        strides[3] = (cuuint64_t)H * W * ld * 2;
    } else {
        SNN_REQUIRE(!hnw, "make_act_map: (h, n, w) order is for plain views only");
        SNN_REQUIRE(H % 2 == 0 && W % 2 == 0, "stride-2 / transposed conv needs even H, W (got %dx%d)", H, W);
        SNN_REQUIRE(C % 64 == 0, "stride-2 / transposed conv needs C %% 64 == 0 (got %d)", C);
        dims[0] = ld + C; dims[1] = W / 2; dims[2] = 2; dims[3] = H / 2; dims[4] = NB;
        strides[0] = 2 * ld * 2; strides[1] = (cuuint64_t)W * ld * 2; strides[2] = (cuuint64_t)2 * W * ld * 2;
        strides[3] = (cuuint64_t)H * W * ld * 2;
    }
    CUresult r = g_encode(m, CU_TENSOR_MAP_DATA_TYPE_BFLOAT16, 5, const_cast<void*>(ptr), dims, strides, box, es,
                          CU_TENSOR_MAP_INTERLEAVE_NONE, CU_TENSOR_MAP_SWIZZLE_128B, CU_TENSOR_MAP_L2_PROMOTION_L2_256B,
                          CU_TENSOR_MAP_FLOAT_OOB_FILL_NONE);
    SNN_REQUIRE(r == CUDA_SUCCESS, "cuTensorMapEncodeTiled(act) failed: %d (NB=%d H=%d W=%d C=%d ld=%lld phase=%d box=%d,%d,%d)",
                (int)r, NB, H, W, C, ld, phase_view, box_n, box_h, box_w);
    return 0;
}

static int make_w_map(CUtensorMap* m, const void* ptr, int wN, int wT, int wK, int box_n) {
    if (t_plan.active) return 0;
    if (get_encode()) return 2;
    SNN_REQUIRE(((uintptr_t)ptr & 15) == 0, "weight pointer must be 16-byte aligned");
    SNN_REQUIRE(wK % 8 == 0, "weight K extent must be a multiple of 8 (got %d)", wK);
    cuuint64_t dims[3] = {(cuuint64_t)wK, (cuuint64_t)wT, (cuuint64_t)wN};
    cuuint64_t strides[2] = {(cuuint64_t)wK * 2, (cuuint64_t)wT * wK * 2};
    cuuint32_t box[3] = {64, 1, (cuuint32_t)box_n}, es[3] = {1, 1, 1};
    CUresult r = g_encode(m, CU_TENSOR_MAP_DATA_TYPE_BFLOAT16, 3, const_cast<void*>(ptr), dims, strides, box, es,
                          CU_TENSOR_MAP_INTERLEAVE_NONE, CU_TENSOR_MAP_SWIZZLE_128B, CU_TENSOR_MAP_L2_PROMOTION_L2_256B,
                          CU_TENSOR_MAP_FLOAT_OOB_FILL_NONE);
    SNN_REQUIRE(r == CUDA_SUCCESS, "cuTensorMapEncodeTiled(weight) failed: %d (N=%d T=%d K=%d box_n=%d)", (int)r, wN, wT, wK, box_n);
    return 0;
}

static int make_out_map(CUtensorMap* m, void* ptr, int f32, int NB, int Ho, int Wo, int n_store, long long ld, int os,
                        int sbw, int sbh, int sbn, int hnw = 0) {
    if (t_plan.active) return 0;
    if (get_encode()) return 2;
    const cuuint64_t es = f32 ? 4 : 2;
    cuuint64_t dims[5], strides[4];
    cuuint32_t box[5] = {(cuuint32_t)(f32 ? 32 : 64), (cuuint32_t)sbw, 1, (cuuint32_t)sbh, (cuuint32_t)sbn}, est[5] = {1, 1, 1, 1, 1};
    if (os == 1 && hnw) {
        dims[0] = n_store; dims[1] = Wo; dims[2] = 1; dims[3] = NB; dims[4] = Ho;
        strides[0] = ld * es; strides[1] = (cuuint64_t)Wo * ld * es; strides[2] = (cuuint64_t)Ho * Wo * ld * es;
        strides[3] = (cuuint64_t)Wo * ld * es;
        box[3] = (cuuint32_t)sbn; box[4] = (cuuint32_t)sbh;
    } else if (os == 1) {
        dims[0] = n_store; dims[1] = Wo; dims[2] = 1; dims[3] = Ho; dims[4] = NB;
        strides[0] = ld * es; strides[1] = (cuuint64_t)Wo * ld * es; strides[2] = (cuuint64_t)Wo * ld * es;
        strides[3] = (cuuint64_t)Ho * Wo * ld * es;
    } else {
        dims[0] = ld + n_store; dims[1] = Wo / 2; dims[2] = 2; dims[3] = Ho / 2; dims[4] = NB;
        strides[0] = 2 * ld * es; strides[1] = (cuuint64_t)Wo * ld * es; strides[2] = (cuuint64_t)2 * Wo * ld * es;
        strides[3] = (cuuint64_t)Ho * Wo * ld * es;
    }
    CUresult r = g_encode(m, f32 ? CU_TENSOR_MAP_DATA_TYPE_FLOAT32 : CU_TENSOR_MAP_DATA_TYPE_BFLOAT16, 5, ptr, dims, strides, box, est,
                          CU_TENSOR_MAP_INTERLEAVE_NONE, CU_TENSOR_MAP_SWIZZLE_128B, CU_TENSOR_MAP_L2_PROMOTION_NONE,
                          CU_TENSOR_MAP_FLOAT_OOB_FILL_NONE);
    SNN_REQUIRE(r == CUDA_SUCCESS, "cuTensorMapEncodeTiled(out) failed: %d (NB=%d Ho=%d Wo=%d C=%d ld=%lld os=%d box=%d,%d,%d)",
                (int)r, NB, Ho, Wo, n_store, ld, os, sbw, sbh, sbn);
    return 0;
}

static int pow2_ceil(int v) { int p = 1; while (p < v) p <<= 1; return p; }

static void pick_box(int NB, int H, int W, int npix, int* bn, int* bh, int* bw) {
    double best = -1;
    for (int w = npix; w >= 1; w >>= 1) {
        if (w > 256) continue;
        for (int h = npix / w; h >= 1; h >>= 1) {
            const int n = npix / (w * h);
            if (w > pow2_ceil(W) || h > pow2_ceil(H)) continue;
            if (n > 256) continue;
            const double ew = (double)W / (((W + w - 1) / w) * w), eh = (double)H / (((H + h - 1) / h) * h),
                         en = (double)NB / (((NB + n - 1) / n) * n);
            const double e = ew * eh * en + 1e-6 * w;
            if (e > best) { best = e; *bn = n; *bh = h; *bw = w; }
        }
    }
}

enum { GEOM_3x3_S1 = 0, GEOM_3x3_S2 = 1, GEOM_1x1 = 2, GEOM_T2x2_S2 = 3 };

struct DebugFlag {
    std::atomic<int> v{0};
    operator int() const { return v.load(std::memory_order_relaxed); }
};
static DebugFlag g_debug_flags[16];
void neuron_debug_set(int k, int v);
void debug_set(int k, int v) {
#ifndef SNN_TIMING_KNOBS
    if (k == 7) return;
#endif
    if ((k >= 0 && k < 8) || (k >= 12 && k < 16)) g_debug_flags[k].v.store(v, std::memory_order_relaxed);
    else if (k >= 8 && k < 12) neuron_debug_set(k - 8, v);
}

static int smem_budget() { return 220 * 1024; }

constexpr int kSchedPairs = 4096;
static unsigned int* g_sched_pool[64];
static std::atomic<unsigned int> g_sched_next{0};
static std::atomic<int> g_dynamic_tiles{0};
void set_dynamic_tiles(int on) { g_dynamic_tiles.store(on ? 1 : 0, std::memory_order_relaxed); }
static int sched_counters(unsigned int** out) {
    *out = nullptr;
    if (!g_dynamic_tiles.load(std::memory_order_relaxed)) return 0;
    const int dev = current_device();
    SNN_REQUIRE(dev >= 0 && dev < 64, "bad CUDA device %d", dev);
    static PerDeviceOnce once;
    SNN_CUDA_OK(once.run([dev] {
        cudaError_t e = cudaMalloc(&g_sched_pool[dev], sizeof(unsigned int) * 2 * kSchedPairs);
        if (e == cudaSuccess) e = cudaMemset(g_sched_pool[dev], 0, sizeof(unsigned int) * 2 * kSchedPairs);
        return e;
    }));
    *out = g_sched_pool[dev] + 2 * (g_sched_next.fetch_add(1u, std::memory_order_relaxed) % kSchedPairs);
    return 0;
}

static int make_w_map(CUtensorMap* m, const void* ptr, int wN, int wT, int wK, int box_n);
struct WDesc { const void* ptr; int wN, wT, wK; };

static bool pair_possible(const ConvGemmParams& p) {
    const int m_tiles = p.tiles_w * p.tiles_h * p.tiles_n;
    if (m_tiles < 2 || g_debug_flags[6] == 1) return false;
    return p.b_mn ? (p.BN % 128 == 0) : (p.BN % 16 == 0);
}

static bool strip_mode_ok(const ConvGemmParams& p) {
    if (g_debug_flags[12] == 1) return false;
    if ((p.bn * p.bw) % 8 != 0) return false;
    if (p.bh < 8 && p.tiles_h == 1) return false;
    if (g_debug_flags[12] == 3 && p.bn != 1) return false;
    const int bn_cta = pair_possible(p) ? p.BN / 2 : p.BN;
    const int b_bytes = p.b_mn ? ((bn_cta + 63) / 64) * 8192 : bn_cta * 128;
    const int chunk = (p.bh + 2) * p.bn * p.bw * 128 + 3 * b_bytes;
    const int stages = (220 * 1024 - 4 * 2 * 4096) / chunk;
    return stages >= (g_debug_flags[12] == 2 ? 3 : 2);
}

static int launch_conv_gemm(const CUtensorMap& a0, const CUtensorMap& a1, const WDesc& wd, ConvGemmParams& p, cudaStream_t st) {
    static PerDeviceOnce once;
    if (!t_plan.active) {
        SNN_CUDA_OK(once.run([] {
            cudaError_t e = cudaFuncSetAttribute(conv_gemm_kernel<false>, cudaFuncAttributeMaxDynamicSharedMemorySize, 226 * 1024);
            if (e == cudaSuccess) e = cudaFuncSetAttribute(conv_gemm_kernel<true>, cudaFuncAttributeMaxDynamicSharedMemorySize, 226 * 1024);
            return e;
        }));
    }
    const int m_tiles = p.tiles_w * p.tiles_h * p.tiles_n;
    bool pair = pair_possible(p);
    if (p.ksplit < 1) p.ksplit = 1;
    const bool strip = p.ntap > 1;
    if (!strip) { p.ntap = 1; p.tap_wstep = 0; }
    int chunks_per_item = 0;
    for (int i = 0; i < p.phase[0].nseg; ++i) chunks_per_item += p.phase[0].seg[i].nchunk * p.ntap;
    chunks_per_item /= p.ksplit;
    const bool small_k = chunks_per_item <= 8;
    if (small_k && g_debug_flags[6] != 2) pair = false;
    SNN_REQUIRE(!(strip && small_k), "conv_gemm: row-strip mode on a small-K conv");
    const int bn_cta = pair ? p.BN / 2 : p.BN;
    p.b_boxes = (bn_cta + 63) / 64;
    p.b_bytes = p.b_mn ? p.b_boxes * 8192 : bn_cta * 128;
    p.a_bytes = strip ? (p.bh + 2) * p.bn * p.bw * 128 : 16384;
    p.a_tap_off = strip ? p.bn * p.bw * 128 : 0;
    p.hnw = strip ? 1 : 0;
    p.chunk_bytes = p.a_bytes + p.ntap * p.b_bytes;
    p.cps = (small_k || strip) ? 1 : (p.BN > 128 ? 1 : (p.BN > 64 ? 2 : 4));
    for (int ph = 0; ph < p.nphase && p.cps > 1; ++ph)
        for (int i = 0; i < p.phase[ph].nseg; ++i)
            while (p.cps > 1 && p.phase[ph].seg[i].nchunk % p.cps != 0) p.cps >>= 1;
    if (g_debug_flags[2] > 0) p.cps = g_debug_flags[2];
    const int es = p.out_f32 ? 4 : 2, CH = p.out_f32 ? 32 : 64;
    char* obase = reinterpret_cast<char*>(p.out) + (long long)p.out_coff * es;
    p.tma_out = g_debug_flags[0] != 1 && ((uintptr_t)obase % 16 == 0) && ((p.out_ld * es) % 16 == 0) &&
                (p.os == 1 || (p.n_store % CH == 0 && p.Ho % 2 == 0 && p.Wo % 2 == 0));
    SNN_REQUIRE(!p.stats || p.tma_out, "conv_fprop: fused statistics need the TMA-store epilogue (output alignment)");
    p.nbuf = 2;
    p.epi_groups = (small_k && g_debug_flags[3] != 1) ? 2 : 1;
    const int stage_extra = p.tma_out ? 4 * p.epi_groups * p.nbuf * 4096 : 0;
    while (p.cps > 1 && (smem_budget() - stage_extra) / (p.cps * p.chunk_bytes) < 3) p.cps >>= 1;
    p.stage_bytes = p.cps * p.chunk_bytes;
    int stages = (smem_budget() - stage_extra) / p.stage_bytes;
    if (stages > kMaxStages) stages = kMaxStages;
    if (g_debug_flags[1] > 0 && stages > g_debug_flags[1]) stages = g_debug_flags[1];
    SNN_REQUIRE(stages >= 2, "conv_gemm: not enough shared memory for 2 stages");
    p.stages = stages;
    const size_t smem = (size_t)stages * p.stage_bytes + stage_extra + 1024;
    p.n_blocks = (p.n_store + p.BN - 1) / p.BN;
    if (sched_counters(&p.sched)) return 2;
#ifdef SNN_TIMING_KNOBS
    p.dbg = g_debug_flags[7];
#else
    p.dbg = 0;
#endif
    if (t_plan.active) {
        const int tiles = (pair ? (m_tiles + 1) / 2 : m_tiles) * p.n_blocks * p.nphase * p.ksplit;
        const int workers = pair ? num_sms() / 2 : num_sms();
        const int v[20] = {p.bn, p.bh, p.bw, p.BN, pair ? 1 : 0, p.ntap > 1 ? 1 : 0, p.hnw, p.stages, p.stage_bytes, p.cps, p.ksplit,
                           tiles, p.n_blocks, workers < tiles ? workers : tiles, p.epi_groups, small_k ? 1 : 0, p.tma_out, (int)smem,
                           p.a_bytes, p.b_bytes};
        for (int i = 0; i < 20; ++i) t_plan.v[i] = v[i];
        return 0;
    }
    CUtensorMap b, o;
    if (make_w_map(&b, wd.ptr, wd.wN, wd.wT, wd.wK, p.b_mn ? 64 : bn_cta)) return 2;
    if (p.tma_out) {
        const int sbw = p.bw >= 32 ? 32 : p.bw;
        int sbh, sbn;
        if (p.hnw) { sbn = (32 / sbw) < p.bn ? (32 / sbw) : p.bn; sbh = 32 / (sbw * sbn); }
        else { sbh = (32 / sbw) < p.bh ? (32 / sbw) : p.bh; sbn = 32 / (sbw * sbh); }
        if (make_out_map(&o, obase, p.out_f32, p.NB, p.Ho, p.Wo, p.n_store, p.out_ld, p.os, sbw, sbh, sbn, p.hnw)) return 2;
    } else {
        o = b;
    }
    if (!pair) {
        const int total_tiles = m_tiles * p.n_blocks * p.nphase * p.ksplit;
        int grid = num_sms();
        if (g_debug_flags[5] > 0) grid = g_debug_flags[5];
        if (grid > total_tiles) grid = total_tiles;
        return check_cuda(launch_pdl(conv_gemm_kernel<false>, dim3(grid), dim3(64 + 128 * p.epi_groups), smem, st, a0, a1, b, o, p),
                          "conv_gemm_kernel launch");
    }
    const int total_tiles = ((m_tiles + 1) / 2) * p.n_blocks * p.nphase * p.ksplit;
    int pairs = num_sms() / 2;
    if (g_debug_flags[5] > 0) pairs = g_debug_flags[5];
    if (pairs > total_tiles) pairs = total_tiles;
    cudaLaunchConfig_t cfg;
    memset(&cfg, 0, sizeof(cfg));
    cfg.gridDim = dim3(2 * pairs, 1, 1);
    cfg.blockDim = dim3(64 + 128 * p.epi_groups, 1, 1);
    cfg.dynamicSmemBytes = smem;
    cfg.stream = st;
    cudaLaunchAttribute attr[2];
    attr[0].id = cudaLaunchAttributeClusterDimension;
    attr[0].val.clusterDim.x = 2; attr[0].val.clusterDim.y = 1; attr[0].val.clusterDim.z = 1;
    attr[1].id = cudaLaunchAttributeProgrammaticStreamSerialization;
    attr[1].val.programmaticStreamSerializationAllowed = 1;
    cfg.attrs = attr;
    cfg.numAttrs = pdl_enabled() ? 2 : 1;
    return check_cuda(cudaLaunchKernelEx(&cfg, conv_gemm_kernel<true>, a0, a1, b, o, p), "conv_gemm_kernel<pair> launch");
}

static int pick_bn(int n_store) {
    if (n_store <= 256) return ((n_store + 15) / 16) * 16;
    int best = 256; double beste = -1;
    for (int bn = 256; bn >= 64; bn -= 16) {
        const int tiles = (n_store + bn - 1) / bn;
        const double e = (double)n_store / (tiles * bn) + 1e-4 * bn / 256.0;
        if (e > beste) { beste = e; best = bn; }
    }
    return best;
}

static void set_domain(ConvGemmParams& p, int NB, int Hd, int Wd, int nb_for_box = 0) {
    p.NB = NB; p.Hd = Hd; p.Wd = Wd;
    pick_box(nb_for_box > 0 ? nb_for_box : NB, Hd, Wd, 128, &p.bn, &p.bh, &p.bw);
    p.tiles_w = (Wd + p.bw - 1) / p.bw; p.tiles_h = (Hd + p.bh - 1) / p.bh; p.tiles_n = (NB + p.bn - 1) / p.bn;
}

static Seg mkseg(int src, int dc, int dw, int dhp, int dh, int wtap, int wc0, int C) {
    Seg s; s.src = src; s.dc = dc; s.dw = dw; s.dhp = dhp; s.dh = dh; s.wtap = wtap; s.wc0 = wc0; s.nchunk = (C + 63) / 64;
    return s;
}

static void s2_tap(int k, int* phase, int* d) {
    if (k == 0) { *phase = 1; *d = -1; } else if (k == 1) { *phase = 0; *d = 0; } else { *phase = 1; *d = 0; }
}

long long conv_stats_groups(int geom, int NB, int H, int W, int B, int* groups_per_t) {
    if (geom != GEOM_3x3_S1 && geom != GEOM_3x3_S2 && geom != GEOM_1x1) return 0;
    if (B <= 0 || NB % B != 0) return 0;
    int Hd = H, Wd = W;
    if (geom == GEOM_3x3_S2) { Hd = H / 2; Wd = W / 2; }
    ConvGemmParams p;
    set_domain(p, NB, Hd, Wd, B);
    if (p.bn > 1 && B % p.bn != 0) return 0;
    const int tiles_hw = p.tiles_w * p.tiles_h;
    if (groups_per_t) *groups_per_t = 4 * (B / p.bn) * tiles_hw;
    return 4LL * tiles_hw * p.tiles_n;
}

int conv_fprop(int geom, int NB, int H, int W, const void* x0, int C0, long long ld0, const void* x1, int C1, long long ld1,
               const void* w, int w_rows, int w_K, int w_coff, int Cout, int w_row_off, const float* bias, void* out,
               int out_f32, long long out_ld, int out_coff, int accumulate, cudaStream_t st, float* stats, int frames_per_step) {
    SNN_REQUIRE(Cout % 8 == 0, "conv_fprop: Cout=%d must be a multiple of 8", Cout);
    ConvGemmParams p;
    memset(&p, 0, sizeof(p));
    p.stats = stats;
    const int taps = geom == GEOM_3x3_S1 || geom == GEOM_3x3_S2 ? 9 : (geom == GEOM_1x1 ? 1 : 4);
    const int phase_view = geom == GEOM_3x3_S2;
    int Hd = H, Wd = W;
    p.os = 1; p.Ho = H; p.Wo = W;
    if (geom == GEOM_3x3_S2) { Hd = H / 2; Wd = W / 2; p.Ho = Hd; p.Wo = Wd; }
    if (geom == GEOM_T2x2_S2) { p.os = 2; p.Ho = 2 * H; p.Wo = 2 * W; }
    set_domain(p, NB, Hd, Wd, stats ? frames_per_step : 0);
    p.BN = pick_bn(Cout);
    p.n_store = Cout; p.wn_off = w_row_off;
    p.out = out; p.bias = bias; p.out_f32 = out_f32; p.accumulate = accumulate; p.out_ld = out_ld; p.out_coff = out_coff;
    const bool strip = geom == GEOM_3x3_S1 && strip_mode_ok(p);
    const int box_h = strip ? p.bh + 2 : p.bh;
    CUtensorMap a0, a1;
    if (make_act_map(&a0, x0, NB, H, W, C0, ld0, phase_view, p.bn, box_h, p.bw, strip)) return 2;
    if (x1) { if (make_act_map(&a1, x1, NB, H, W, C1, ld1, phase_view, p.bn, box_h, p.bw, strip)) return 2; } else a1 = a0;
    const WDesc wd = {w, w_rows, taps, w_K};
    if (stats) {
        int gpt = 0;
        SNN_REQUIRE(conv_stats_groups(geom, NB, H, W, frames_per_step, &gpt) > 0 && out_f32 && !accumulate && !bias && out_coff == 0,
                    "conv_fprop: fused BatchNorm statistics are not available for this call (geom %d NB %d %dx%d B %d)", geom,
                    NB, H, W, frames_per_step);
    }
    if (geom == GEOM_T2x2_S2) {
        p.nphase = 4;
        for (int a = 0; a < 2; ++a)
            for (int bb = 0; bb < 2; ++bb) {
                Phase& ph = p.phase[a * 2 + bb];
                ph.oph = a; ph.opw = bb; ph.nseg = 0;
                ph.seg[ph.nseg++] = mkseg(0, 0, 0, 0, 0, a * 2 + bb, w_coff, C0);
                if (x1) ph.seg[ph.nseg++] = mkseg(1, 0, 0, 0, 0, a * 2 + bb, w_coff + C0, C1);
            }
    } else if (strip) {
        p.nphase = 1; p.ntap = 3; p.tap_wstep = 3;
        Phase& ph = p.phase[0];
        ph.nseg = 0;
        for (int kw = 0; kw < 3; ++kw) {
            ph.seg[ph.nseg++] = mkseg(0, 0, kw - 1, 0, -1, kw, w_coff, C0);
            if (x1) ph.seg[ph.nseg++] = mkseg(1, 0, kw - 1, 0, -1, kw, w_coff + C0, C1);
        }
    } else {
        p.nphase = 1;
        Phase& ph = p.phase[0];
        ph.nseg = 0;
        const int k = geom == GEOM_1x1 ? 1 : 3;
        for (int kh = 0; kh < k; ++kh)
            for (int kw = 0; kw < k; ++kw) {
                int dcm = 0, dw = 0, dhp = 0, dh = 0;
                if (geom == GEOM_3x3_S1) { dw = kw - 1; dh = kh - 1; }
                if (geom == GEOM_3x3_S2) { int pc; s2_tap(kh, &dhp, &dh); s2_tap(kw, &pc, &dw); dcm = pc; }
                ph.seg[ph.nseg++] = mkseg(0, (int)(dcm * ld0), dw, dhp, dh, kh * k + kw, w_coff, C0);
                if (x1) ph.seg[ph.nseg++] = mkseg(1, (int)(dcm * ld1), dw, dhp, dh, kh * k + kw, w_coff + C0, C1);
            }
    }
    return launch_conv_gemm(a0, a1, wd, p, st);
}

int conv_dgrad(int geom, int NB, int H, int W, const void* dy, int Cout, long long ld_dy, const void* wt, int w_K,
               int ci_off, int Ci, void* dx, int dx_f32, long long dx_ld, int dx_coff, int accumulate, cudaStream_t st) {
    SNN_REQUIRE(Ci % 8 == 0, "conv_dgrad: Ci=%d must be a multiple of 8", Ci);
    ConvGemmParams p;
    memset(&p, 0, sizeof(p));
    const int taps = geom == GEOM_3x3_S1 || geom == GEOM_3x3_S2 ? 9 : (geom == GEOM_1x1 ? 1 : 4);
    int Hd = H, Wd = W, Hy = H, Wy = W, phase_view = 0;
    p.os = 1; p.Ho = H; p.Wo = W;
    if (geom == GEOM_3x3_S2) { Hd = H / 2; Wd = W / 2; Hy = Hd; Wy = Wd; p.os = 2; }
    if (geom == GEOM_T2x2_S2) { Hy = 2 * H; Wy = 2 * W; phase_view = 1; }
    set_domain(p, NB, Hd, Wd);
    p.BN = pick_bn(Ci);
    p.n_store = Ci; p.wn_off = ci_off; p.b_mn = 1;
    p.out = dx; p.bias = nullptr; p.out_f32 = dx_f32; p.accumulate = accumulate; p.out_ld = dx_ld; p.out_coff = dx_coff;
    int ks = 1;
    if (dx_f32 && !accumulate && geom != GEOM_3x3_S2 && dx_coff == 0 && dx_ld == Ci && g_debug_flags[0] != 1) {
        const int m_work = (p.tiles_w * p.tiles_h * p.tiles_n + 1) / 2;
        const int items = m_work * ((Ci + p.BN - 1) / p.BN);
        const int nseg = taps, pairs = num_sms() / 2;
        for (int cand = 1; cand <= nseg; ++cand)
            if (nseg % cand == 0 && items * cand <= 2 * pairs) ks = cand;
        if (!(ks > 1 && items <= pairs / 2)) ks = 1;
    }
    if (deterministic()) ks = 1;
    const bool strip = ks == 1 && geom == GEOM_3x3_S1 && strip_mode_ok(p);
    CUtensorMap a0;
    if (make_act_map(&a0, dy, NB, Hy, Wy, Cout, ld_dy, phase_view, p.bn, strip ? p.bh + 2 : p.bh, p.bw, strip)) return 2;
    const WDesc wd = {wt, Cout, taps, w_K};
    if (strip) {
        p.nphase = 1; p.ntap = 3; p.tap_wstep = -3;
        Phase& ph = p.phase[0];
        for (int kw = 0; kw < 3; ++kw) ph.seg[ph.nseg++] = mkseg(0, 0, 1 - kw, 0, -1, 6 + kw, 0, Cout);
    } else if (geom == GEOM_3x3_S1 || geom == GEOM_1x1) {
        p.nphase = 1;
        Phase& ph = p.phase[0];
        const int k = geom == GEOM_1x1 ? 1 : 3;
        for (int kh = 0; kh < k; ++kh)
            for (int kw = 0; kw < k; ++kw)
                ph.seg[ph.nseg++] = mkseg(0, 0, k == 3 ? 1 - kw : 0, 0, k == 3 ? 1 - kh : 0, kh * k + kw, 0, Cout);
    } else if (geom == GEOM_3x3_S2) {
        p.nphase = 4;
        for (int pr = 0; pr < 2; ++pr)
            for (int pc = 0; pc < 2; ++pc) {
                Phase& ph = p.phase[pr * 2 + pc];
                ph.oph = pr; ph.opw = pc; ph.nseg = 0;
                for (int kh = 0; kh < 3; ++kh) {
                    if ((kh == 1) != (pr == 0)) continue;
                    const int dh = kh == 0 ? 1 : 0;
                    for (int kw = 0; kw < 3; ++kw) {
                        if ((kw == 1) != (pc == 0)) continue;
                        const int dw = kw == 0 ? 1 : 0;
                        ph.seg[ph.nseg++] = mkseg(0, 0, dw, 0, dh, kh * 3 + kw, 0, Cout);
                    }
                }
            }
    } else {
        p.nphase = 1;
        Phase& ph = p.phase[0];
        for (int a = 0; a < 2; ++a)
            for (int bb = 0; bb < 2; ++bb) ph.seg[ph.nseg++] = mkseg(0, (int)(bb * ld_dy), 0, a, 0, a * 2 + bb, 0, Cout);
    }
    if (ks > 1) {
        if (!t_plan.active) SNN_CUDA_OK(cudaMemsetAsync(dx, 0, sizeof(float) * (size_t)NB * H * W * Ci, st));
        p.ksplit = ks;
        p.accumulate = 1;
    }
    return launch_conv_gemm(a0, a0, wd, p, st);
}

int conv_wgrad(int geom, int NB, int H, int W, const void* x, int Ci, long long ld_x, const void* dy, int Cout,
               long long ld_dy, float* dw, int w_K, int w_coff, cudaStream_t st) {
    static PerDeviceOnce once;
    if (!t_plan.active) {
        SNN_CUDA_OK(once.run([] {
            cudaError_t e = cudaFuncSetAttribute(wgrad_gemm_kernel<false>, cudaFuncAttributeMaxDynamicSharedMemorySize, 226 * 1024);
            if (e == cudaSuccess) e = cudaFuncSetAttribute(wgrad_gemm_kernel<true>, cudaFuncAttributeMaxDynamicSharedMemorySize, 226 * 1024);
            return e;
        }));
    }
    SNN_REQUIRE(Ci % 8 == 0 && Cout % 8 == 0 && w_K % 4 == 0 && w_coff % 4 == 0, "conv_wgrad: channel counts must be multiples of 8");
    WgradParams p;
    memset(&p, 0, sizeof(p));
    const int taps = geom == GEOM_3x3_S1 || geom == GEOM_3x3_S2 ? 9 : (geom == GEOM_1x1 ? 1 : 4);
    int Hd = H, Wd = W, Hy = H, Wy = W, x_phase = 0, g_phase = 0;
    if (geom == GEOM_3x3_S2) { Hd = H / 2; Wd = W / 2; Hy = Hd; Wy = Wd; x_phase = 1; }
    if (geom == GEOM_T2x2_S2) { Hy = 2 * H; Wy = 2 * W; g_phase = 1; }
    p.NB = NB; p.Hd = Hd; p.Wd = Wd;
    pick_box(NB, Hd, Wd, 64, &p.bn, &p.bh, &p.bw);
    p.tiles_w = (Wd + p.bw - 1) / p.bw; p.tiles_h = (Hd + p.bh - 1) / p.bh; p.tiles_n = (NB + p.bn - 1) / p.bn;
    p.total_tiles = p.tiles_w * p.tiles_h * p.tiles_n;
    {
        const int c64 = (Ci + 63) / 64;
        int nt = c64 >= 4 ? 4 : c64;
        if (c64 > 4) {
            for (int cand = 4; cand >= 2; --cand) if (c64 % cand == 0) { nt = cand; break; }
        }
        p.NT = nt * 64;
        p.n_ci_tiles = (Ci + p.NT - 1) / p.NT;
    }
    p.Cout = Cout; p.Ci = Ci; p.dw = dw; p.dw_ld = (long long)taps * w_K; p.wK = w_K; p.w_coff = w_coff;
    p.strip = geom == GEOM_3x3_S1 && (p.bn * p.bw) % 8 == 0 && (Ci % 128 == 0 || Ci == 64) && g_debug_flags[13] != 1 &&
              (p.bh >= 8 || p.tiles_h > 1) &&
              !(g_debug_flags[13] == 2 && p.bn != 1);
    if (p.strip) {
        p.NT = Ci == 64 ? 64 : 128;
        p.n_ci_tiles = (Ci + p.NT - 1) / p.NT;
        p.x_box_bytes = (p.bh + 2) * p.bn * p.bw * 128;
        p.x_tap_off = p.bn * p.bw * 128;
        p.hnw = 1;
    }
    const bool pair = Cout > 128 && p.NT % 128 == 0 && g_debug_flags[6] != 1;
    p.stage_bytes = p.strip ? 2 * 8192 + ((pair ? p.NT / 2 : p.NT) / 64) * p.x_box_bytes : (2 + (pair ? p.NT / 2 : p.NT) / 64) * 8192;
    const int stage_extra = 4 * 8192;
    int stages = (smem_budget() - stage_extra) / p.stage_bytes;
    if (stages > kMaxStages) stages = kMaxStages;
    p.stages = stages;
    p.lbo_bytes = 8192;
    p.sbo_bytes = 1024;
    p.ntaps = p.strip ? 3 : taps;
    const int k = geom == GEOM_1x1 ? 1 : (geom == GEOM_T2x2_S2 ? 2 : 3);
    if (p.strip) {
        for (int kw = 0; kw < 3; ++kw) {
            WTap& t = p.taps[kw];
            memset(&t, 0, sizeof(t));
            t.wtap = kw; t.x_dw = kw - 1; t.x_dh = -1;
        }
    } else
    for (int kh = 0; kh < k; ++kh)
        for (int kw = 0; kw < k; ++kw) {
            WTap& t = p.taps[kh * k + kw];
            memset(&t, 0, sizeof(t));
            t.wtap = kh * k + kw;
            if (geom == GEOM_3x3_S1) { t.x_dw = kw - 1; t.x_dh = kh - 1; }
            if (geom == GEOM_3x3_S2) { int pc; s2_tap(kh, &t.x_dhp, &t.x_dh); s2_tap(kw, &pc, &t.x_dw); t.x_dc = (int)(pc * ld_x); }
            if (geom == GEOM_T2x2_S2) { t.g_dhp = kh; t.g_dc = (int)(kw * ld_dy); }
        }
    p.m_items = pair ? (Cout + 255) / 256 : (Cout + 127) / 128;
    const int base = p.m_items * p.n_ci_tiles * p.ntaps;
    const int workers = pair ? num_sms() / 2 : num_sms();
    int ksplit = 1;
    if (base < workers) {
        const int k2 = (2 * workers) / base, k1 = workers / base;
        ksplit = (k2 >= 1 && p.total_tiles / k2 >= 16) ? k2 : (k1 >= 1 ? k1 : 1);
        if (p.strip && k1 >= 1 && g_debug_flags[14] != 1) ksplit = k1;
    }
    const int max_split = (p.total_tiles + 3) / 4;
    if (ksplit > max_split) ksplit = max_split;
    if (ksplit < 1) ksplit = 1;
    if (g_debug_flags[4] > 0) ksplit = g_debug_flags[4];
    if (deterministic()) ksplit = 1;
    p.tiles_per_split = (p.total_tiles + ksplit - 1) / ksplit;
    p.ksplit = (p.total_tiles + p.tiles_per_split - 1) / p.tiles_per_split;
    CUtensorMap mg, mx, mw;
    if (make_act_map(&mg, dy, NB, Hy, Wy, Cout, ld_dy, g_phase, p.bn, p.bh, p.bw, p.hnw)) return 2;
    if (make_act_map(&mx, x, NB, H, W, Ci, ld_x, x_phase, p.bn, p.strip ? p.bh + 2 : p.bh, p.bw, p.hnw)) return 2;
    if (!t_plan.active) {
        if (get_encode()) return 2;
        SNN_REQUIRE(((uintptr_t)dw & 15) == 0, "conv_wgrad: dw must be 16-byte aligned");
        cuuint64_t dims[3] = {(cuuint64_t)w_K, (cuuint64_t)taps, (cuuint64_t)Cout};
        cuuint64_t strides[2] = {(cuuint64_t)w_K * 4, (cuuint64_t)taps * w_K * 4};
        cuuint32_t box[3] = {32, 1, 32}, es[3] = {1, 1, 1};
        CUresult r = g_encode(&mw, CU_TENSOR_MAP_DATA_TYPE_FLOAT32, 3, dw, dims, strides, box, es, CU_TENSOR_MAP_INTERLEAVE_NONE,
                              CU_TENSOR_MAP_SWIZZLE_128B, CU_TENSOR_MAP_L2_PROMOTION_NONE, CU_TENSOR_MAP_FLOAT_OOB_FILL_NONE);
        SNN_REQUIRE(r == CUDA_SUCCESS, "cuTensorMapEncodeTiled(dw) failed: %d (Cout=%d taps=%d K=%d)", (int)r, Cout, taps, w_K);
    }
    const size_t smem = (size_t)p.stages * p.stage_bytes + stage_extra + 1024;
    if (sched_counters(&p.sched)) return 2;
    const int items = base * p.ksplit;
    int nw = workers < items ? workers : items;
    if (g_debug_flags[5] > 0 && nw > g_debug_flags[5]) nw = g_debug_flags[5];
    if (t_plan.active) {
        const int v[20] = {p.bn, p.bh, p.bw, p.NT, pair ? 1 : 0, p.strip, p.hnw, p.stages, p.stage_bytes, 1, p.ksplit, items, p.n_ci_tiles, nw, 1, 0, 1,
                           (int)smem, p.strip ? p.x_box_bytes : 8192, 2 * 8192};
        for (int i = 0; i < 20; ++i) t_plan.v[i] = v[i];
        return 0;
    }
    if (!pair) {
        return check_cuda(launch_pdl(wgrad_gemm_kernel<false>, dim3(nw), dim3(192), smem, st, mg, mx, mw, p), "wgrad_gemm_kernel launch");
    }
    cudaLaunchConfig_t cfg;
    memset(&cfg, 0, sizeof(cfg));
    cfg.gridDim = dim3(2 * nw, 1, 1);
    cfg.blockDim = dim3(192, 1, 1);
    cfg.dynamicSmemBytes = smem;
    cfg.stream = st;
    cudaLaunchAttribute attr[2];
    attr[0].id = cudaLaunchAttributeClusterDimension;
    attr[0].val.clusterDim.x = 2; attr[0].val.clusterDim.y = 1; attr[0].val.clusterDim.z = 1;
    attr[1].id = cudaLaunchAttributeProgrammaticStreamSerialization;
    attr[1].val.programmaticStreamSerializationAllowed = 1;
    cfg.attrs = attr;
    cfg.numAttrs = pdl_enabled() ? 2 : 1;
    return check_cuda(cudaLaunchKernelEx(&cfg, wgrad_gemm_kernel<true>, mg, mx, mw, p), "wgrad_gemm_kernel<pair> launch");
}

int conv_plan(int kind, int geom, int NB, int H, int W, int Cin, int Cout, int out_f32, int frames_per_step, int accumulate, int* out) {
    void* const dummy = reinterpret_cast<void*>((uintptr_t)1 << 20);
    t_plan.active = true;
    for (int i = 0; i < 24; ++i) t_plan.v[i] = 0;
    int rc;
    if (kind == 0)
        rc = conv_fprop(geom, NB, H, W, dummy, Cin, Cin, nullptr, 0, 0, dummy, Cout, Cin, 0, Cout, 0, nullptr, dummy, out_f32, Cout, 0, accumulate,
                        nullptr, frames_per_step > 0 ? static_cast<float*>(dummy) : nullptr, frames_per_step);
    else if (kind == 1)
        rc = conv_dgrad(geom, NB, H, W, dummy, Cout, Cout, dummy, Cin, 0, Cin, dummy, out_f32, Cin, 0, accumulate, nullptr);
    else
        rc = conv_wgrad(geom, NB, H, W, dummy, Cin, Cin, dummy, Cout, Cout, static_cast<float*>(dummy), Cin, 0, nullptr);
    t_plan.active = false;
    if (rc == 0) for (int i = 0; i < 20; ++i) out[i] = t_plan.v[i];
    return rc;
}

}
```

### snn_object_detectionddp_b200/kernels.py

```python
import torch

from . import _lib
from ._lib import (ACT_LIF, ACT_SILU, GEOM_1x1, GEOM_3x3_S1, GEOM_3x3_S2, GEOM_T2x2_S2, GEOM_TAPS, call, ptr,
                   require_cuda, stream_ptr)


def _nhwc_ld(x):
    nb, h, w, c = x.shape
    ld = x.stride(2) if w > 1 else (x.stride(1) if h > 1 else (x.stride(0) if nb > 1 else c))
    if x.stride(3) != 1 and c > 1:
        raise ValueError("NHWC view must be channel-contiguous")
    if (w > 1 and x.stride(2) != ld) or (h > 1 and x.stride(1) != w * ld) or (nb > 1 and x.stride(0) != h * w * ld):
        raise ValueError(f"not a dense NHWC pixel grid: shape {tuple(x.shape)} strides {x.stride()}")
    return ld


def out_hw(geom, h, w):
    if geom == GEOM_3x3_S2:
        return h // 2, w // 2
    if geom == GEOM_T2x2_S2:
        return 2 * h, 2 * w
    return h, w


def _conv_flops(geom, nb, h, w, cin, cout):
    ho, wo = out_hw(geom, h, w)
    if geom == GEOM_T2x2_S2:
        return 2.0 * nb * h * w * cout * cin * 4
    return 2.0 * nb * ho * wo * cout * cin * GEOM_TAPS[geom]


def conv_fprop(geom, x0, w_bf16, cout, x1=None, bias=None, out=None, out_dtype=torch.float32, w_coff=0, w_row_off=0,
               accumulate=False):
    require_cuda(x0, x1, w_bf16, bias, out)
    nb, h, w, c0 = x0.shape
    ho, wo = out_hw(geom, h, w)
    if out is None:
        out = torch.empty((nb, ho, wo, cout), device=x0.device, dtype=out_dtype)
    assert x0.dtype == torch.bfloat16 and w_bf16.dtype == torch.bfloat16 and w_bf16.is_contiguous()
    assert tuple(out.shape) == (nb, ho, wo, cout)
    rows, taps, wk = w_bf16.shape
    assert taps == GEOM_TAPS[geom]
    c1 = 0 if x1 is None else x1.shape[3]
    if x1 is not None:
        assert x1.dtype == torch.bfloat16 and tuple(x1.shape[:3]) == (nb, h, w)
    assert w_coff + c0 + c1 <= wk and w_row_off + cout <= rows
    call("snn_conv_fprop", geom, nb, h, w, ptr(x0), c0, _nhwc_ld(x0), ptr(x1), c1, 0 if x1 is None else _nhwc_ld(x1),
         ptr(w_bf16), rows, wk, w_coff, cout, w_row_off, ptr(bias), ptr(out), int(out.dtype == torch.float32),
         _nhwc_ld(out), 0, int(accumulate), stream_ptr(), work=("flop", _conv_flops(geom, nb, h, w, c0 + c1, cout), f"g{geom} nb{nb} {h}x{w} {c0 + c1}->{cout}"))
    return out


_STATS_GROUPS = {}


def conv_fprop_partials(geom, x0, w_bf16, cout, T, x1=None):
    require_cuda(x0, x1, w_bf16)
    nb, h, w, c0 = x0.shape
    key = (geom, nb, h, w, T)
    if key not in _STATS_GROUPS:
        gpt = _lib.ctypes.c_int(0)
        n = _lib.lib().snn_conv_stats_groups(geom, nb, h, w, nb // T, _lib.ctypes.byref(gpt)) if nb % T == 0 else 0
        _STATS_GROUPS[key] = (int(n), int(gpt.value))
    groups, gpt = _STATS_GROUPS[key]
    if groups == 0:
        return conv_fprop(geom, x0, w_bf16, cout, x1=x1), None, 0
    ho, wo = out_hw(geom, h, w)
    out = torch.empty((nb, ho, wo, cout), device=x0.device, dtype=torch.float32)
    rows, taps, wk = w_bf16.shape
    c1 = 0 if x1 is None else x1.shape[3]
    assert x0.dtype == torch.bfloat16 and w_bf16.dtype == torch.bfloat16 and w_bf16.is_contiguous() and taps == GEOM_TAPS[geom]
    assert c0 + c1 <= wk and cout <= rows
    part = torch.empty((groups, 2, cout), device=x0.device, dtype=torch.float32)
    call("snn_conv_fprop_stats", geom, nb, h, w, ptr(x0), c0, _nhwc_ld(x0), ptr(x1), c1, 0 if x1 is None else _nhwc_ld(x1),
         ptr(w_bf16), rows, wk, 0, cout, 0, ptr(out), nb // T, ptr(part), stream_ptr(),
         work=("flop", _conv_flops(geom, nb, h, w, c0 + c1, cout), f"g{geom} nb{nb} {h}x{w} {c0 + c1}->{cout}"))
    return out, part, gpt


def conv_fprop_stats(geom, x0, w_bf16, cout, T, x1=None):
    out, part, gpt = conv_fprop_partials(geom, x0, w_bf16, cout, T, x1=x1)
    if part is None:
        return out, None
    sums = torch.empty((T, 2, cout), device=x0.device, dtype=torch.float64)
    call("snn_bn_stats_from_partials", ptr(part), ptr(sums), T, cout, gpt, stream_ptr(), work=("byte", 4.0 * part.numel()))
    return out, sums


def bn_finalize_partials(part, gpt, gamma, beta, running_mean, running_var, num_batches_tracked, counters, T, C, P, eps, momentum):
    require_cuda(part, gamma, beta, running_mean, running_var, num_batches_tracked, counters)
    dev = part.device
    scale, shift, mean, invstd = (torch.empty((T, C), device=dev, dtype=torch.float32) for _ in range(4))
    sums = torch.empty((T, 2, C), device=dev, dtype=torch.float64)
    ws = torch.empty((int(_lib.lib().snn_bn_finalize_workspace_doubles(T, C, gpt)),), device=dev, dtype=torch.float64)
    assert counters.dtype == torch.int32 and counters.numel() >= (C + 31) // 32
    assert num_batches_tracked is None or num_batches_tracked.dtype == torch.int64
    call("snn_bn_finalize_partials", ptr(part), ptr(sums), ptr(ws), ptr(gamma), ptr(beta), ptr(running_mean), ptr(running_var),
         ptr(num_batches_tracked), ptr(scale), ptr(shift), ptr(mean), ptr(invstd), ptr(counters), T, C, P, gpt, float(eps),
         float(momentum), stream_ptr(), work=("byte", 4.0 * part.numel()))
    return scale, shift, mean, invstd


def conv_dgrad(geom, dy, w_bf16, in_hw, ci, ci_off=0, out=None, out_dtype=torch.bfloat16, accumulate=False):
    require_cuda(dy, w_bf16, out)
    nb, hy, wy, cout = dy.shape
    h, w = in_hw
    assert out_hw(geom, h, w) == (hy, wy), (geom, in_hw, dy.shape)
    rows, taps, wk = w_bf16.shape
    assert taps == GEOM_TAPS[geom] and rows == cout and ci_off + ci <= wk
    assert dy.dtype == torch.bfloat16 and w_bf16.dtype == torch.bfloat16 and w_bf16.is_contiguous()
    if out is None:
        out = torch.empty((nb, h, w, ci), device=dy.device, dtype=out_dtype)
    call("snn_conv_dgrad", geom, nb, h, w, ptr(dy), cout, _nhwc_ld(dy), ptr(w_bf16), wk, ci_off, ci, ptr(out),
         int(out.dtype == torch.float32), _nhwc_ld(out), 0, int(accumulate), stream_ptr(),
         work=("flop", _conv_flops(geom, nb, h, w, ci, cout), f"g{geom} nb{nb} {h}x{w} {ci}<-{cout}"))
    return out


def conv_wgrad(geom, x, dy, dw, w_coff=0):
    require_cuda(x, dy, dw)
    nb, h, w, ci = x.shape
    cout = dy.shape[3]
    assert tuple(dy.shape[:3]) == (nb,) + out_hw(geom, h, w)
    rows, taps, wk = dw.shape
    assert rows == cout and taps == GEOM_TAPS[geom] and w_coff + ci <= wk
    assert dw.dtype == torch.float32 and dw.is_contiguous() and x.dtype == torch.bfloat16 and dy.dtype == torch.bfloat16
    call("snn_conv_wgrad", geom, nb, h, w, ptr(x), ci, _nhwc_ld(x), ptr(dy), cout, _nhwc_ld(dy), ptr(dw), wk, w_coff,
         stream_ptr(), work=("flop", _conv_flops(geom, nb, h, w, ci, cout), f"g{geom} nb{nb} {h}x{w} {ci}x{cout}"))
    return dw


PLAN_FIELDS = ("bn", "bh", "bw", "n_tile", "pair", "strip", "hnw", "stages", "stage_bytes", "chunks_per_stage", "ksplit", "items",
               "n_blocks", "ctas", "epi_groups", "small_k", "tma_out", "smem_bytes", "a_bytes", "b_bytes")


def conv_plan(kind, geom, nb, h, w, cin, cout, out_f32=True, frames_per_step=0, accumulate=False):
    import ctypes
    out = (ctypes.c_int * 20)()
    rc = _lib.lib().snn_conv_plan({"fprop": 0, "dgrad": 1, "wgrad": 2}[kind], geom, nb, h, w, cin, cout, int(out_f32), frames_per_step,
                             int(accumulate), out)
    if rc:
        raise _lib.SnnKernelError(f"snn_conv_plan failed (rc={rc}): {_lib.lib().snn_last_error().decode()}")
    return dict(zip(PLAN_FIELDS, list(out)))


def weight_prep(w_master, want_fprop=True, want_dgrad=True, wf=None, wt=None):
    require_cuda(w_master)
    n, t, k = w_master.shape
    assert w_master.is_contiguous() and w_master.dtype == torch.float32
    if want_fprop and wf is None:
        wf = torch.empty((n, t, k), device=w_master.device, dtype=torch.bfloat16)
    if want_dgrad and wt is None:
        wt = torch.empty((k, t, n), device=w_master.device, dtype=torch.bfloat16)
    call("snn_weight_prep", ptr(w_master), ptr(wf), ptr(wt), n, t, k, stream_ptr())
    return wf, wt


def bn_stats(y, T):
    require_cuda(y)
    c = y.shape[-1]
    p = y.numel() // (T * c)
    sums = torch.empty((T, 2, c), device=y.device, dtype=torch.float64)
    ws = torch.empty((int(_lib.lib().snn_bn_stats_workspace_floats(T, p, c)),), device=y.device, dtype=torch.float32)
    call("snn_bn_stats", ptr(y), ptr(sums), ptr(ws), T, p, c, stream_ptr(), work=("byte", 4.0 * y.numel()))
    return sums


def bn_finalize(sums, gamma, beta, running_mean, running_var, T, C, P, eps, momentum, training):
    require_cuda(sums, gamma, beta, running_mean, running_var)
    dev = gamma.device
    n = T if training else 1
    scale, shift, mean, invstd = (torch.empty((n, C), device=dev, dtype=torch.float32) for _ in range(4))
    call("snn_bn_finalize", ptr(sums), ptr(gamma), ptr(beta), ptr(running_mean), ptr(running_var), ptr(scale), ptr(shift),
         ptr(mean), ptr(invstd), T, C, P, float(eps), float(momentum), int(training), stream_ptr())
    return scale, shift, mean, invstd


def bn_act_fwd(act, y, scale, shift, T, v_init=None, want_mask=True, want_v_final=False, beta=0.5, theta=1.0):
    require_cuda(y, scale, shift, v_init)
    c = y.shape[-1]
    n_per_t = y.numel() // T
    out = torch.empty(y.shape, device=y.device, dtype=torch.bfloat16)
    mask = torch.empty((T, n_per_t // 8), device=y.device, dtype=torch.uint8) if (want_mask and act == ACT_LIF) else None
    v_final = torch.empty((n_per_t,), device=y.device, dtype=torch.float32) if want_v_final else None
    ss = c if scale.shape[0] == T and scale.dim() == 2 and scale.shape[0] > 1 else 0
    if scale.dim() == 2 and scale.shape[0] == 1:
        ss = 0
    if T == 1:
        ss = 0
    nbytes = y.numel() * (6.0 + (0.125 if mask is not None else 0.0))
    nbytes += (0 if v_init is None else 4.0 * n_per_t) + (0 if v_final is None else 4.0 * n_per_t)
    call("snn_bn_act_fwd", act, ptr(y), ptr(scale), ptr(shift), ptr(v_init), ptr(out), ptr(mask), ptr(v_final), T, n_per_t,
         c, ss, float(beta), float(theta), stream_ptr(), work=("byte", nbytes, f"T{T} n{n_per_t} C{c}"))
    return out, mask, v_final


def bn_act_bwd(act, training, y, scale, shift, mean, invstd, gs, T, v_init=None, gv_final=None, want_gv_init=False,
               beta=0.5, theta=1.0, alpha=2.0):
    require_cuda(y, scale, shift, mean, invstd, gs, v_init, gv_final)
    c = y.shape[-1]
    p = y.numel() // (T * c)
    dev = y.device
    gx = torch.empty(y.shape, device=dev, dtype=torch.float32) if training else None
    dy = None if training else torch.empty(y.shape, device=dev, dtype=torch.bfloat16)
    red = torch.empty((T, 2, c), device=dev, dtype=torch.float32) if training else None
    gv_init = torch.empty((p * c,), device=dev, dtype=torch.float32) if want_gv_init else None
    ss = 0 if (T == 1 or scale.shape[0] == 1) else c
    assert gs.dtype == torch.bfloat16 and gs.is_contiguous()
    nbytes = y.numel() * (10.0 if training else 8.0)
    call("snn_bn_act_bwd", act, int(training), ptr(y), ptr(scale), ptr(shift), ptr(mean), ptr(invstd), ptr(v_init), ptr(gs),
         ptr(gv_final), ptr(gx), ptr(dy), ptr(gv_init), ptr(red), T, p, c, ss, float(beta), float(theta), float(alpha),
         stream_ptr(), work=("byte", nbytes))
    return gx, dy, gv_init, red


def bn_act_bwd_train(act, y, scale, shift, mean, invstd, beta_bn, gs, T, dgamma, dbeta, v_init=None, gv_final=None,
                     want_gv_init=False, beta=0.5, theta=1.0, alpha=2.0):
    require_cuda(y, scale, shift, mean, invstd, beta_bn, gs, dgamma, dbeta, v_init, gv_final)
    c = y.shape[-1]
    p = y.numel() // (T * c)
    dev = y.device
    assert gs.dtype == torch.bfloat16 and gs.is_contiguous() and y.is_contiguous()
    assert scale.shape[0] == T and mean.shape[0] == T
    red = torch.empty((T, 2, c), device=dev, dtype=torch.float32)
    dy = torch.empty(y.shape, device=dev, dtype=torch.bfloat16)
    gv_init = torch.empty((p * c,), device=dev, dtype=torch.float32) if want_gv_init else None
    args = (ptr(y), ptr(scale), ptr(shift), ptr(mean), ptr(invstd), ptr(beta_bn), ptr(v_init), ptr(gs), ptr(gv_final), ptr(red),
            ptr(dy), ptr(gv_init), ptr(dgamma), ptr(dbeta), T, p, c, float(beta), float(theta), float(alpha), stream_ptr())
    tag = f"T{T} n{p * c} C{c}"
    call("snn_bn_act_bwd2", 0, act, *args, work=("byte", 6.0 * y.numel(), "reduce " + tag))
    call("snn_bn_act_bwd2", 1, act, *args, work=("byte", 8.0 * y.numel(), "dx " + tag))
    return dy, gv_init, red


def bn_bwd_dx(red, gamma, gx, y, scale, mean, invstd, dgamma, dbeta, T):
    require_cuda(red, gamma, gx, y, scale, mean, invstd, dgamma, dbeta)
    c = y.shape[-1]
    p = y.numel() // (T * c)
    coef = torch.empty((T, 2, c), device=y.device, dtype=torch.float32)
    dy = torch.empty(y.shape, device=y.device, dtype=torch.bfloat16)
    call("snn_bn_bwd_dx", ptr(red), ptr(gamma), ptr(gx), ptr(y), ptr(scale), ptr(mean), ptr(invstd), ptr(coef), ptr(dgamma),
         ptr(dbeta), ptr(dy), T, p, c, stream_ptr(), work=("byte", 10.0 * y.numel()))
    return dy


def lstm_gates_fwd(gates, c_prev, ch, h_bf16_out=None, c_out=None):
    require_cuda(gates, c_prev, h_bf16_out, c_out)
    p = gates.numel() // (4 * ch)
    shape = gates.shape[:-1] + (ch,)
    c_next = torch.empty(shape, device=gates.device, dtype=torch.float32) if c_out is None else c_out
    h_next = torch.empty(shape, device=gates.device, dtype=torch.float32)
    h_bf16 = torch.empty(shape, device=gates.device, dtype=torch.bfloat16) if h_bf16_out is None else h_bf16_out
    assert gates.is_contiguous() and c_next.is_contiguous() and h_bf16.is_contiguous()
    call("snn_lstm_gates_fwd", ptr(gates), ptr(c_prev), ptr(c_next), ptr(h_next), ptr(h_bf16), p, ch, stream_ptr())
    return h_next, c_next, h_bf16


def lstm_gates_bwd(gates, c_prev, c_next, dh, dc_in, ch, dgates_out=None, dh_bf16=None):
    require_cuda(gates, c_prev, c_next, dh, dh_bf16, dc_in, dgates_out)
    p = gates.numel() // (4 * ch)
    dgates = torch.empty(gates.shape, device=gates.device, dtype=torch.bfloat16) if dgates_out is None else dgates_out
    assert gates.is_contiguous() and dgates.is_contiguous()
    assert dh is None or (dh.is_contiguous() and dh.dtype == torch.float32)
    assert dh_bf16 is None or (dh_bf16.is_contiguous() and dh_bf16.dtype == torch.bfloat16)
    dc_prev = torch.empty(c_next.shape, device=gates.device, dtype=torch.float32)
    call("snn_lstm_gates_bwd", ptr(gates), ptr(c_prev), ptr(c_next), ptr(dh), ptr(dh_bf16), ptr(dc_in), ptr(dgates), ptr(dc_prev), p, ch,
         stream_ptr())
    return dgates, dc_prev


def nchw_to_nhwc(x, dtype=torch.bfloat16, out=None):
    require_cuda(x)
    nb, c, h, w = x.shape
    x = x.contiguous()
    if out is None:
        out = torch.empty((nb, h, w, c), device=x.device, dtype=dtype)
    call("snn_nchw_to_nhwc", ptr(x), ptr(out), int(out.dtype == torch.bfloat16), nb, c, h * w, _nhwc_ld(out), 0, stream_ptr())
    return out


def nhwc_to_nchw(x):
    require_cuda(x)
    nb, h, w, c = x.shape
    out = torch.empty((nb, c, h, w), device=x.device, dtype=torch.float32)
    call("snn_nhwc_to_nchw", ptr(x), int(x.dtype == torch.bfloat16), ptr(out), nb, c, h * w, _nhwc_ld(x), 0, stream_ptr())
    return out


def bilinear_resize(x, out_hw):
    require_cuda(x)
    nb, hi, wi, c = x.shape
    ho, wo = out_hw
    assert x.is_contiguous() and x.dtype == torch.bfloat16
    y = torch.empty((nb, ho, wo, c), device=x.device, dtype=torch.bfloat16)
    call("snn_bilinear_resize", 0, ptr(x), ptr(y), nb, hi, wi, ho, wo, c, stream_ptr(),
         work=("byte", 2.0 * (x.numel() + y.numel())))
    return y


def bilinear_resize_bwd(gy, in_hw):
    require_cuda(gy)
    nb, ho, wo, c = gy.shape
    hi, wi = in_hw
    assert gy.is_contiguous() and gy.dtype == torch.bfloat16
    gx = torch.empty((nb, hi, wi, c), device=gy.device, dtype=torch.bfloat16)
    call("snn_bilinear_resize", 1, ptr(gy), ptr(gx), nb, hi, wi, ho, wo, c, stream_ptr(),
         work=("byte", 2.0 * (gx.numel() + gy.numel())))
    return gx


def pad_crop(x, out_hw):
    require_cuda(x)
    nb, hs, ws, c = x.shape
    hd, wd = out_hw
    assert x.is_contiguous() and x.dtype == torch.bfloat16
    y = torch.empty((nb, hd, wd, c), device=x.device, dtype=torch.bfloat16)
    call("snn_nhwc_pad_crop", ptr(x), ptr(y), nb, hs, ws, hd, wd, c, stream_ptr(), work=("byte", 2.0 * (x.numel() + y.numel())))
    return y


def colsum_accumulate(dy, acc):
    require_cuda(dy, acc)
    c = dy.shape[-1]
    assert dy.is_contiguous() and dy.dtype == torch.bfloat16 and acc.numel() == c and acc.is_contiguous()
    call("snn_colsum_bf16", ptr(dy), ptr(acc), dy.numel() // c, c, stream_ptr())


def grad_sumsq(g, acc, zero_first=True):
    require_cuda(g, acc)
    call("snn_grad_sumsq", ptr(g), g.numel(), ptr(acc), int(zero_first), stream_ptr(), work=("byte", 4.0 * g.numel()))


def adamw_step(p, g, m, v, shadow, hp, sumsq, gnorm_out=None, step=None, zero_grad=False):
    require_cuda(p, g, m, v, shadow, hp, sumsq, gnorm_out, step)
    n_rows = hp.shape[0] if (step is not None and hp.dim() == 2) else 1
    call("snn_adamw_step", ptr(p), ptr(g), ptr(m), ptr(v), ptr(shadow), p.numel(), ptr(hp), ptr(sumsq), ptr(gnorm_out),
         ptr(step), n_rows, int(bool(zero_grad)), stream_ptr(),
         work=("byte", (28.0 + (2.0 if shadow is not None else 0.0)) * p.numel()))


GEOM_DW3x3 = 4


def dw3x3_fprop(x, w9c, T=0):
    require_cuda(x, w9c)
    nb, h, w, c = x.shape
    assert x.is_contiguous() and x.dtype == torch.bfloat16 and w9c.is_contiguous() and w9c.numel() == 9 * c
    y = torch.empty((nb, h, w, c), device=x.device, dtype=torch.float32)
    nbytes = 6.0 * y.numel()
    if T and nb % T == 0:
        gpt = int(_lib.lib().snn_dw3x3_stats_blocks(nb // T, w, c))
        part = torch.empty((T, gpt, 2, c), device=x.device, dtype=torch.float32)
        call("snn_dw3x3_fprop_stats", ptr(x), ptr(w9c), ptr(y), nb, h, w, c, T, ptr(part), stream_ptr(),
             work=("byte", nbytes, f"dw fwd+stats nb{nb} {h}x{w} C{c}"))
        return y, part, gpt
    call("snn_dw3x3_fprop", ptr(x), ptr(w9c), ptr(y), nb, h, w, c, stream_ptr(), work=("byte", nbytes, f"dw fwd nb{nb} {h}x{w} C{c}"))
    return (y, None, 0) if T else y


def dw3x3_dgrad(dy, w9c, out=None):
    require_cuda(dy, w9c, out)
    nb, h, w, c = dy.shape
    assert dy.is_contiguous() and dy.dtype == torch.bfloat16
    dx = torch.empty((nb, h, w, c), device=dy.device, dtype=torch.bfloat16) if out is None else out
    assert dx.is_contiguous() and tuple(dx.shape) == (nb, h, w, c) and dx.dtype == torch.bfloat16
    call("snn_dw3x3_dgrad", ptr(dy), ptr(w9c), ptr(dx), nb, h, w, c, stream_ptr(), work=("byte", 4.0 * dy.numel(), f"dw dgrad nb{nb} {h}x{w} C{c}"))
    return dx


def dw3x3_wgrad(x, dy, dw9c):
    require_cuda(x, dy, dw9c)
    nb, h, w, c = x.shape
    assert x.is_contiguous() and dy.is_contiguous() and dw9c.is_contiguous() and dw9c.dtype == torch.float32
    call("snn_dw3x3_wgrad", ptr(x), ptr(dy), ptr(dw9c), nb, h, w, c, stream_ptr(), work=("byte", 4.0 * x.numel(), f"dw wgrad nb{nb} {h}x{w} C{c}"))


def space_to_depth8(frames, B, T):
    require_cuda(frames)
    assert frames.is_contiguous() and frames.dtype in (torch.float32, torch.uint8)
    h, w = frames.shape[-2:]
    out = torch.empty((T * B, h // 8, w // 8, 192), device=frames.device, dtype=torch.bfloat16)
    name = "snn_space_to_depth8" if frames.dtype == torch.float32 else "snn_space_to_depth8_u8"
    call(name, ptr(frames), ptr(out), B, T, h, w, stream_ptr())
    return out


def detect_decode(distri, scores, anchors, stride, xywh, want_probs=True):
    require_cuda(distri, scores, anchors, stride)
    b, a, r4 = distri.shape
    nc = scores.shape[2]
    assert distri.is_contiguous() and scores.is_contiguous() and distri.dtype == torch.float32 and scores.dtype == torch.float32
    boxes = torch.empty((b, a, 4), device=distri.device, dtype=torch.float32)
    probs = torch.empty((b, a, nc), device=distri.device, dtype=torch.float32) if want_probs else None
    call("snn_detect_decode", ptr(distri), ptr(scores), ptr(anchors), ptr(stride), b, a, nc, r4 // 4, int(xywh), ptr(boxes),
         ptr(probs), stream_ptr())
    return boxes, probs


def _a_off_arg(a_off):
    if not a_off:
        return 0, None
    arr = (_lib.ctypes.c_int * len(a_off))(*[int(v) for v in a_off])
    return len(a_off) - 1, arr


def detect_assign_loss_fwd(distri, scores, a_off, anchors, stride, gt_cls, gt_box, gt_valid, img_wh, B, A, nc, reg_max, topk,
                           gains, counter):
    require_cuda(distri, scores, anchors, stride, gt_cls, gt_box, gt_valid, gains, counter)
    dev = distri.device
    M = gt_cls.shape[1]
    assert gt_cls.dtype == torch.int64 and gt_box.dtype == torch.float32 and gt_valid.dtype in (torch.bool, torch.uint8)
    assert gt_cls.is_contiguous() and gt_box.is_contiguous() and gt_valid.is_contiguous() and distri.is_contiguous() and scores.is_contiguous()
    assert tuple(gt_cls.shape) == (B, M) and tuple(gt_box.shape) == (B, M, 4) and distri.numel() == B * A * 4 * reg_max
    assert counter.dtype == torch.int32 and gains.dtype == torch.float32 and gains.numel() == 3
    ws = torch.empty((int(_lib.lib().snn_tal_workspace_bytes(B, A, M)) + 15) // 16 * 4, device=dev, dtype=torch.float32)
    pboxes = torch.empty((B, A, 4), device=dev, dtype=torch.float32)
    probs = torch.empty((B, A, nc), device=dev, dtype=torch.float32)
    tbox = torch.empty((B, A, 4), device=dev, dtype=torch.float32)
    tscores = torch.empty((B, A, nc), device=dev, dtype=torch.float32)
    fg = torch.empty((B, A), device=dev, dtype=torch.uint8)
    sums = torch.empty(3, device=dev, dtype=torch.float64)
    out6 = torch.empty(6, device=dev, dtype=torch.float32)
    coef3 = torch.empty(3, device=dev, dtype=torch.float32)
    nl, arr = _a_off_arg(a_off)
    call("snn_detect_assign_loss_fwd", ptr(distri), ptr(scores), nl, arr, ptr(anchors), ptr(stride), ptr(gt_cls), ptr(gt_box),
         ptr(gt_valid), float(img_wh[0]), float(img_wh[1]), B, A, M, nc, reg_max, int(topk), ptr(gains), ptr(ws), ptr(pboxes),
         ptr(probs), ptr(tbox), ptr(tscores), ptr(fg), ptr(sums), ptr(counter), ptr(out6), ptr(coef3), stream_ptr())
    return out6, coef3, (tbox, tscores, fg)


def tal_assign(probs, pboxes, anchors, stride, gt_cls, gt_box, gt_valid, img_wh, nc, topk=10):
    require_cuda(probs, pboxes, anchors, stride, gt_cls, gt_box, gt_valid)
    B, A = probs.shape[0], probs.shape[1]
    M = gt_cls.shape[1]
    dev = probs.device
    ws = torch.empty((int(_lib.lib().snn_tal_workspace_bytes(B, A, M)) + 15) // 16 * 4, device=dev, dtype=torch.float32)
    tbox = torch.empty((B, A, 4), device=dev, dtype=torch.float32)
    tscores = torch.empty((B, A, nc), device=dev, dtype=torch.float32)
    fg = torch.empty((B, A), device=dev, dtype=torch.uint8)
    assert probs.is_contiguous() and pboxes.is_contiguous() and gt_cls.dtype == torch.int64
    call("snn_tal_assign", ptr(probs), ptr(pboxes), ptr(anchors), ptr(stride), ptr(gt_cls.contiguous()), ptr(gt_box.contiguous()),
         ptr(gt_valid.contiguous()), float(img_wh[0]), float(img_wh[1]), B, A, M, nc, int(topk), ptr(ws), ptr(tbox), ptr(tscores), ptr(fg),
         stream_ptr())
    return tbox, tscores, fg


def detect_loss_bwd_rows(distri, scores, a_off, anchors, stride, targets, B, A, nc, reg_max, coef3, gout3, bf16):
    tbox, tscores, fg = targets
    require_cuda(distri, scores, anchors, stride, tbox, tscores, fg, coef3, gout3)
    dt = torch.bfloat16 if bf16 else torch.float32
    g_distri = torch.empty(distri.shape, device=distri.device, dtype=dt)
    g_scores = torch.empty(scores.shape, device=distri.device, dtype=dt)
    nl, arr = _a_off_arg(a_off)
    assert gout3 is None or (gout3.dtype == torch.float32 and gout3.is_contiguous() and gout3.numel() == 3)
    call("snn_detect_loss_bwd_rows", ptr(distri), ptr(scores), nl, arr, ptr(anchors), ptr(stride), ptr(tbox), ptr(tscores), ptr(fg),
         B, A, nc, reg_max, ptr(coef3), ptr(gout3), ptr(g_distri), ptr(g_scores), int(bf16), stream_ptr())
    return g_distri, g_scores


def detect_loss_fwd(distri, scores, anchors, stride, tbox_px, tscores, fg):
    require_cuda(distri, scores, anchors, stride, tbox_px, tscores, fg)
    b, a, r4 = distri.shape
    sums = torch.empty(3, device=distri.device, dtype=torch.float64)
    for t in (distri, scores, anchors, stride, tbox_px, tscores, fg):
        assert t.is_contiguous()
    assert fg.dtype == torch.uint8 and tscores.dtype == torch.float32 and tbox_px.dtype == torch.float32
    call("snn_detect_loss_fwd", ptr(distri), ptr(scores), ptr(anchors), ptr(stride), ptr(tbox_px), ptr(tscores), ptr(fg), b, a,
         scores.shape[2], r4 // 4, ptr(sums), stream_ptr())
    return sums


def detect_loss_bwd(distri, scores, anchors, stride, tbox_px, tscores, fg, coef):
    require_cuda(distri, scores, anchors, stride, tbox_px, tscores, fg, coef)
    b, a, r4 = distri.shape
    g_distri, g_scores = torch.empty_like(distri), torch.empty_like(scores)
    assert coef.dtype == torch.float32 and coef.is_contiguous() and coef.numel() == 3
    call("snn_detect_loss_bwd", ptr(distri), ptr(scores), ptr(anchors), ptr(stride), ptr(tbox_px), ptr(tscores), ptr(fg), b, a,
         scores.shape[2], r4 // 4, ptr(coef), ptr(g_distri), ptr(g_scores), stream_ptr())
    return g_distri, g_scores
```

Measured before the change: 6765.

## Split last-wave conv GEMM tiles across idle workers with K-partial reduction

Adds a tail-splitting scheduler to the persistent conv GEMM kernel. When the last wave of tiles would leave workers idle, the remaining tiles are split along K into 2-4 parts and assigned to otherwise idle CTAs. Partial accumulators go through a global workspace and are ordered with acquire/release flags and atomic claims. This is meant to reduce wave-quantization imbalance, at the cost of extra scratch traffic, synchronization and a second kernel template instantiation.

After: 6779, median of 6. Within noise of the previous version (+0.2%).

```diff
diff --git a/include/snn_b200.h b/include/snn_b200.h
--- a/include/snn_b200.h
+++ b/include/snn_b200.h
@@ -10,7 +10,8 @@
 void snn_debug_set(int key, int value);
 void snn_set_tile_scheduling(int dynamic);
 int snn_conv_plan(int kind, int geom, int NB, int H, int W, int Cin, int Cout, int out_f32, int frames_per_step, int accumulate,
-                  int* out20);
+                  int* out23);
+int snn_conv_tail_job(int items, int workers, int tail_parts, int worker, int i);
 void snn_set_deterministic(int on);
 int snn_get_deterministic(void);
 void snn_set_dependent_launch(int on);
diff --git a/snn_object_detectionddp_b200/_lib.py b/snn_object_detectionddp_b200/_lib.py
--- a/snn_object_detectionddp_b200/_lib.py
+++ b/snn_object_detectionddp_b200/_lib.py
@@ -63,7 +63,7 @@
 
 
 def exported_symbols():
-    return sorted(list(_SIGNATURES) + ["snn_last_error", "snn_version", "snn_debug_set", "snn_set_tile_scheduling", "snn_set_dependent_launch", "snn_get_dependent_launch", "snn_set_deterministic", "snn_get_deterministic", "snn_conv_plan", "snn_tensor_map_cache_stats", "snn_conv_stats_groups", "snn_bn_stats_workspace_floats", "snn_nms_workspace_keys",
+    return sorted(list(_SIGNATURES) + ["snn_last_error", "snn_version", "snn_debug_set", "snn_set_tile_scheduling", "snn_set_dependent_launch", "snn_get_dependent_launch", "snn_set_deterministic", "snn_get_deterministic", "snn_conv_plan", "snn_conv_tail_job", "snn_tensor_map_cache_stats", "snn_conv_stats_groups", "snn_bn_stats_workspace_floats", "snn_nms_workspace_keys",
                                              "snn_tal_workspace_bytes", "snn_dw3x3_stats_blocks", "snn_bn_finalize_workspace_doubles"])
 
 
@@ -110,6 +110,8 @@
         L.snn_set_dependent_launch(int(os.environ.get("SNN_DEPENDENT_LAUNCH", "0")))
         L.snn_conv_plan.argtypes = [_I] * 10 + [ctypes.POINTER(_I)]
         L.snn_conv_plan.restype = _I
+        L.snn_conv_tail_job.argtypes = [_I] * 5
+        L.snn_conv_tail_job.restype = _I
         L.snn_set_deterministic.argtypes = [_I]
         L.snn_set_deterministic.restype = None
         L.snn_get_deterministic.argtypes = []
diff --git a/snn_object_detectionddp_b200/csrc/api.cu b/snn_object_detectionddp_b200/csrc/api.cu
--- a/snn_object_detectionddp_b200/csrc/api.cu
+++ b/snn_object_detectionddp_b200/csrc/api.cu
@@ -75,6 +75,7 @@
 void set_dynamic_tiles(int on);
 void tmap_cache_stats(unsigned long long*, unsigned long long*);
 int conv_plan(int, int, int, int, int, int, int, int, int, int, int*);
+int conv_tail_job(int, int, int, int, int);
 int conv_fprop(int, int, int, int, const void*, int, long long, const void*, int, long long, const void*, int, int, int, int,
                int, const float*, void*, int, long long, int, int, cudaStream_t, float*, int);
 long long conv_stats_groups(int, int, int, int, int, int*);
@@ -148,8 +149,11 @@
 int snn_version(void) { return 100; }
 void snn_debug_set(int key, int value) { debug_set(key, value); }
 void snn_set_tile_scheduling(int dynamic) { set_dynamic_tiles(dynamic); }
-int snn_conv_plan(int kind, int geom, int NB, int H, int W, int Cin, int Cout, int out_f32, int frames_per_step, int accumulate, int* out20) {
-    return conv_plan(kind, geom, NB, H, W, Cin, Cout, out_f32, frames_per_step, accumulate, out20);
+int snn_conv_plan(int kind, int geom, int NB, int H, int W, int Cin, int Cout, int out_f32, int frames_per_step, int accumulate, int* out23) {
+    return conv_plan(kind, geom, NB, H, W, Cin, Cout, out_f32, frames_per_step, accumulate, out23);
+}
+int snn_conv_tail_job(int items, int workers, int tail_parts, int worker, int i) {
+    return conv_tail_job(items, workers, tail_parts, worker, i);
 }
 void snn_set_deterministic(int on) { set_deterministic(on); }
 int snn_get_deterministic(void) { return deterministic() ? 1 : 0; }
diff --git a/snn_object_detectionddp_b200/csrc/gemm_tc.cu b/snn_object_detectionddp_b200/csrc/gemm_tc.cu
--- a/snn_object_detectionddp_b200/csrc/gemm_tc.cu
+++ b/snn_object_detectionddp_b200/csrc/gemm_tc.cu
@@ -42,6 +42,9 @@
     int dbg;
     int ntap, a_bytes, a_tap_off, b_bytes, tap_wstep;
     int hnw;
+    int tail_q, tail_base, tail_absorb;
+    unsigned int* tail_ctl;
+    float* tail_ws;
     Phase phase[4];
 };
 
@@ -74,9 +77,77 @@
 constexpr int kMaxStages = 8;
 constexpr int kTmemCols = 256;
 
+constexpr int kTailMax = 160;
+constexpr int kTailFlagOff = 4 * kTailMax;
+constexpr int kTailDoneOff = kTailFlagOff + 8 * kTailMax;
+constexpr int kTailCtlWords = kTailDoneOff + 1;
+
+__host__ __device__ constexpr int tail_pattern(int q, int a) {
+#define TE(x, k, pre, i) (((x) | ((k) << 2) | ((pre) << 4)) << (5 * (i)))
+    return q == 2 ? (a == 1 ? TE(0, 0, 1, 0) : TE(0, 1, 0, 0)) | (1 << 15)
+         : q == 3 ? (a == 2 ? TE(0, 0, 1, 0) | TE(1, 1, 1, 1) : a == 1 ? TE(1, 0, 1, 0) | TE(0, 2, 0, 1) : TE(0, 1, 0, 0) | TE(1, 2, 0, 1)) | (2 << 15)
+         : (a == 3 ? TE(0, 0, 1, 0) | TE(1, 1, 1, 1) | TE(2, 1, 1, 2) : a == 2 ? TE(1, 0, 1, 0) | TE(0, 1, 1, 1) | TE(2, 3, 0, 2)
+            : a == 1 ? TE(2, 0, 1, 0) | TE(0, 2, 0, 1) | TE(1, 3, 0, 2) : TE(2, 2, 0, 0) | TE(1, 2, 0, 1) | TE(0, 3, 0, 2)) | (3 << 15);
+#undef TE
+}
+__host__ __device__ inline int tail_split_tiles(int total, int nw, int q, int* base) {
+    const int R = (total + nw - 1) / nw, L = total - (R - 1) * nw;
+    *base = total;
+    if (q < 2 || R < 2 || L >= nw) return 0;
+    const int G = L / (q - 1), r = L % (q - 1);
+    if (G * q + (r ? r + 1 : 0) > nw) return 0;
+    *base = total - L;
+    return L;
+}
+__host__ __device__ inline int tail_parts(int j, int L, int q) {
+    return j < (L / (q - 1)) * (q - 1) ? q : L % (q - 1) + 1;
+}
+__host__ __device__ inline int tail_job(int i, int w, int nw, int total, int q) {
+    int base;
+    const int L = q ? tail_split_tiles(total, nw, q, &base) : 0;
+    if (L == 0) { const int t = w + i * nw; return t < total ? t : -1; }
+    const int G = L / (q - 1), r = L % (q - 1);
+    int qq = 0, a = 0, j0 = 0;
+    if (w / q < G) { qq = q; a = w % q; j0 = (w / q) * (q - 1); }
+    else if (r > 0 && w >= G * q && w <= G * q + r) { qq = r + 1; a = w - G * q; j0 = G * (q - 1); }
+    const int pat = qq ? tail_pattern(qq, a) : 0, n = pat >> 15;
+    int npre = 0;
+    for (int u = 0; u < n; ++u) npre += (pat >> (5 * u + 4)) & 1;
+    const int full = base / nw;
+    int u = -1;
+    if (i < npre) u = i;
+    else if (i < npre + full) return w + (i - npre) * nw;
+    else if (i < n + full) u = i - full;
+    if (u < 0) return -1;
+    const int ent = (pat >> (5 * u)) & 31;
+    return (base + j0 + (ent & 3)) | (((ent >> 2) & 3) << 24);
+}
+SNN_DEVINL void st_release_gpu(unsigned int* a, unsigned int v) {
+    asm volatile("st.release.gpu.global.u32 [%0], %1;" ::"l"(a), "r"(v) : "memory");
+}
+SNN_DEVINL unsigned int ld_acquire_gpu(const unsigned int* a) {
+    unsigned int v;
+    asm volatile("ld.acquire.gpu.global.u32 %0, [%1];" : "=r"(v) : "l"(a) : "memory");
+    return v;
+}
+SNN_DEVINL void tmem_st16(uint32_t taddr, const uint32_t* r) {
+    asm volatile(
+        "tcgen05.st.sync.aligned.32x32b.x16.b32 [%0], "
+        "{%1, %2, %3, %4, %5, %6, %7, %8, %9, %10, %11, %12, %13, %14, %15, %16};"
+        ::"r"(taddr), "r"(r[0]), "r"(r[1]), "r"(r[2]), "r"(r[3]), "r"(r[4]), "r"(r[5]), "r"(r[6]), "r"(r[7]),
+          "r"(r[8]), "r"(r[9]), "r"(r[10]), "r"(r[11]), "r"(r[12]), "r"(r[13]), "r"(r[14]), "r"(r[15])
+        : "memory");
+}
+SNN_DEVINL void tmem_st_wait() { asm volatile("tcgen05.wait::st.sync.aligned;" ::: "memory"); }
+SNN_DEVINL int tile_stages(const Phase& ph, int sg0, int spp, int cps) {
+    int S = 0;
+    for (int sg = sg0; sg < sg0 + spp; ++sg) S += (ph.seg[sg].nchunk + cps - 1) / cps;
+    return S;
+}
+
 constexpr int kAccCols = 256;
 
-template <bool PAIR>
+template <bool PAIR, bool SPLIT>
 __global__ void __launch_bounds__(320, 1)
 conv_gemm_kernel(const __grid_constant__ CUtensorMap tmA0, const __grid_constant__ CUtensorMap tmA1,
                  const __grid_constant__ CUtensorMap tmB, const __grid_constant__ CUtensorMap tmO,
@@ -137,6 +208,27 @@
         uint32_t a_s = sbase;
         const bool dyn = p.sched != nullptr;
         int tile = worker, nxt1 = -1, pend = 0, pub = 0;
+        const bool split = SPLIT;
+        int ji = 0;
+        auto resolve = [&]() -> int {
+            for (;;) {
+                const int jb = tail_job(ji++, worker, nworkers, total_tiles, p.tail_q);
+                if (jb < 0) return -1;
+                const int tl = jb & 0xFFFFFF, k = jb >> 24;
+                if (tl < p.tail_base) return tl;
+                unsigned int* claim = p.tail_ctl + 4 * (tl - p.tail_base);
+                int res = -1;
+                if (lane == 0) {
+                    if (!(p.tail_absorb && k == 0) && atomicCAS(claim + k, 0u, 1u) == 0u) {
+                        int lo = k;
+                        while (lo > 0 && atomicCAS(claim + lo - 1, 0u, 1u) == 0u) --lo;
+                        res = tl | (lo << 24) | (k << 27);
+                    }
+                }
+                res = __shfl_sync(0xffffffffu, res, 0);
+                if (res >= 0) return res;
+            }
+        };
         if (dyn && rank == 0) {
             if (tile >= total_tiles) tile = -1;
             sched_publish<PAIR>(ring, pub++, tile, lead);
@@ -149,9 +241,18 @@
                 if (nxt1 < 0) pub = -1;
                 else if (lane == 0) pend = (int)atomicAdd(p.sched, 1u) + nworkers;
             }
+        } else if (split && rank == 0) {
+            tile = resolve();
+            sched_publish<PAIR>(ring, pub++, tile, lead);
+            if (tile < 0) pub = -1;
+            if (pub > 0) {
+                nxt1 = resolve();
+                sched_publish<PAIR>(ring, pub++, nxt1, lead);
+                if (nxt1 < 0) pub = -1;
+            }
         }
         for (int it = 0;; ++it) {
-            if (!dyn) {
+            if (!dyn && !split) {
                 tile = worker + it * nworkers;
                 if (tile >= total_tiles) break;
             } else if (rank == 0) {
@@ -160,19 +261,28 @@
                 tile = sched_next<PAIR>(ring, it, lane);
                 if (tile < 0) break;
             }
-            const int mt = (tile % m_work) * (PAIR ? 2 : 1) + (int)rank, rest = tile / m_work;
+            const int tl = tile & 0xFFFFFF;
+            const int mt = (tl % m_work) * (PAIR ? 2 : 1) + (int)rank, rest = tl / m_work;
             const int ncol0 = p.wn_off + (rest % p.n_blocks) * p.BN + (int)rank * bn_cta;
             const int pk = rest / p.n_blocks;
             const Phase& ph = p.phase[pk % p.nphase];
             const int tw = mt % p.tiles_w, th = (mt / p.tiles_w) % p.tiles_h, tn = mt / (p.tiles_w * p.tiles_h);
             const int w0 = tw * p.bw, h0 = th * p.bh, n0 = tn * p.bn;
             const int spp = ph.nseg / p.ksplit, sg0 = (pk / p.nphase) * spp;
+            int s_lo = 0, s_hi = 1 << 30;
+            if (SPLIT && tl >= p.tail_base) {
+                const int S = tile_stages(ph, sg0, spp, p.cps), qj = tail_parts(tl - p.tail_base, total_tiles - p.tail_base, p.tail_q);
+                s_lo = ((tile >> 24) & 7) * S / qj;
+                s_hi = (((tile >> 27) & 3) + 1) * S / qj;
+            }
+            int gs = 0;
             for (int sg = sg0; sg < sg0 + spp; ++sg) {
                 const Seg g = ph.seg[sg];
                 const CUtensorMap* tmA = g.src ? &tmA1 : &tmA0;
                 const int cw = w0 + g.dw, chh = h0 + g.dh;
                 int ca = g.dc, cb = g.wc0;
-                for (int kc = 0; kc < g.nchunk; kc += p.cps) {
+                for (int kc = 0; kc < g.nchunk; kc += p.cps, ca += 64 * p.cps, cb += 64 * p.cps, ++gs) {
+                    if (SPLIT && (gs < s_lo || gs >= s_hi)) continue;
                     const int nsub = min(p.cps, g.nchunk - kc);
                     mbar_wait(smem_u32(&empty_bar[s]), par ^ 1u);
                     if (lead) {
@@ -216,7 +326,6 @@
                             }
                         }
                     }
-                    ca += 64 * p.cps; cb += 64 * p.cps;
                     a_s += stage_bytes;
                     if (++s == stages) { s = 0; par ^= 1u; a_s = sbase; }
                 }
@@ -229,6 +338,15 @@
                     sched_publish<PAIR>(ring, pub++, nxt1, lead);
                     if (nxt1 < 0) pub = -1;
                     else if (lane == 0) pend = (int)atomicAdd(p.sched, 1u) + nworkers;
+                } else {
+                    nxt1 = -1;
+                }
+            } else if (split && rank == 0) {
+                tile = nxt1;
+                if (pub > 0) {
+                    nxt1 = resolve();
+                    sched_publish<PAIR>(ring, pub++, nxt1, lead);
+                    if (nxt1 < 0) pub = -1;
                 } else {
                     nxt1 = -1;
                 }
@@ -250,22 +368,32 @@
             int s = 0, lt = 0;
             uint32_t par = 0;
             uint32_t a_s = sbase;
-            const bool dyn = p.sched != nullptr;
+            const bool use_ring = SPLIT || p.sched != nullptr;
             for (;; ++lt) {
-                const int tile = dyn ? sched_next<PAIR>(ring, lt, lane) : (worker + lt * nworkers < total_tiles ? worker + lt * nworkers : -1);
-                if (tile < 0) break;
+                const int job = use_ring ? sched_next<PAIR>(ring, lt, lane) : (worker + lt * nworkers < total_tiles ? worker + lt * nworkers : -1);
+                if (job < 0) break;
+                const int tile = job & 0xFFFFFF;
                 const int pk = (tile / m_work) / p.n_blocks;
                 const Phase& ph = p.phase[pk % p.nphase];
                 const int spp = ph.nseg / p.ksplit, sg0 = (pk / p.nphase) * spp;
+                const int S = SPLIT ? tile_stages(ph, sg0, spp, p.cps) : 0;
+                int s_lo = 0, s_hi = S;
+                if (SPLIT && tile >= p.tail_base) {
+                    const int qj = tail_parts(tile - p.tail_base, total_tiles - p.tail_base, p.tail_q);
+                    s_lo = ((job >> 24) & 7) * S / qj;
+                    s_hi = (((job >> 27) & 3) + 1) * S / qj;
+                }
                 const int acc = lt & 1;
-                mbar_wait(smem_u32(&tmem_empty_bar[acc]), (uint32_t)(((lt >> 1) & 1) ^ 1));
+                mbar_wait(smem_u32(&tmem_empty_bar[acc]), (uint32_t)(((lt >> 1) & 1) ^ (SPLIT ? 0 : 1)));
                 tc_fence_after();
                 const uint32_t tacc = tmem_base + (uint32_t)(acc * kAccCols);
-                uint32_t first = 1u;
+                uint32_t first = s_lo == 0 ? 1u : 0u;
+                int gs = 0;
                 for (int sg = sg0; sg < sg0 + spp; ++sg) {
                     const int nchunk = ph.seg[sg].nchunk;
                     const bool last_seg = sg == sg0 + spp - 1;
-                    for (int kc = 0; kc < nchunk; kc += p.cps) {
+                    for (int kc = 0; kc < nchunk; kc += p.cps, ++gs) {
+                        if (SPLIT && (gs < s_lo || gs >= s_hi)) continue;
                         const int nsub = min(p.cps, nchunk - kc);
                         mbar_wait(smem_u32(&full_bar[s]), par);
                         tc_fence_after();
@@ -288,7 +416,7 @@
                                 }
                             }
                             if (PAIR) umma_commit_pair(smem_u32(&empty_bar[s])); else umma_commit(smem_u32(&empty_bar[s]));
-                            if (last_seg && kc + p.cps >= nchunk) {
+                            if (SPLIT ? gs == s_hi - 1 : (last_seg && kc + p.cps >= nchunk)) {
                                 if (PAIR) umma_commit_pair(smem_u32(&tmem_full_bar[acc])); else umma_commit(smem_u32(&tmem_full_bar[acc]));
                             }
                         }
@@ -305,12 +433,62 @@
         const int row = q * 32 + lane;
         const int wl = row % p.bw;
         const int hl = p.hnw ? row / (p.bw * p.bn) : (row / p.bw) % p.bh, nl = p.hnw ? (row / p.bw) % p.bn : row / (p.bw * p.bh);
-        int lt = 0;
         uint32_t gcc = 0;
-        const bool dyn = p.sched != nullptr;
-        for (;; ++lt) {
-            const int tile = dyn ? sched_next<PAIR>(ring, lt, lane) : (worker + lt * nworkers < total_tiles ? worker + lt * nworkers : -1);
-            if (tile < 0) break;
+        const bool use_ring = SPLIT || p.sched != nullptr;
+        const int n_split = total_tiles - p.tail_base;
+        auto job_at = [&](int i) -> int {
+            return use_ring ? sched_next<PAIR>(ring, i, lane) : (worker + i * nworkers < total_tiles ? worker + i * nworkers : -1);
+        };
+        auto part_ws = [&](int j) -> float4* {
+            return reinterpret_cast<float4*>(p.tail_ws) + (size_t)((j * (PAIR ? 2 : 1) + (int)rank) * 4 + q) * (size_t)(p.BN / 4) * 32u;
+        };
+        auto part_flag = [&](int j) -> unsigned int* { return p.tail_ctl + kTailFlagOff + (j * 2 + (int)rank) * 4 + q; };
+        auto has_pred = [&](int v) { return SPLIT && (v & 0xFFFFFF) >= p.tail_base && ((v >> 24) & 7) > 0; };
+        auto is_source = [&](int v) {
+            return SPLIT && (v & 0xFFFFFF) >= p.tail_base &&
+                   ((v >> 27) & 3) + 1 < tail_parts((v & 0xFFFFFF) - p.tail_base, n_split, p.tail_q);
+        };
+        auto prep = [&](int jn, int v) {
+            if (has_pred(v)) {
+                const int j = (v & 0xFFFFFF) - p.tail_base;
+                const unsigned int need = (unsigned int)((v >> 24) & 7);
+                if (lane == 0) {
+                    uint32_t spins = 0;
+                    while (ld_acquire_gpu(part_flag(j)) < need) {
+                        __nanosleep(128);
+                        if (++spins > (1u << 26)) __trap();
+                    }
+                }
+                __syncwarp();
+                __threadfence();
+                const float4* src = part_ws(j);
+                const uint32_t tb = tmem_base + (uint32_t)((jn & 1) * kAccCols) + ((uint32_t)(q * 32) << 16);
+                for (int c = 0; c < p.BN; c += 16) {
+                    uint32_t r[16];
+#pragma unroll
+                    for (int u = 0; u < 4; ++u) {
+                        const float4 t = __ldcg(src + (size_t)(c / 4 + u) * 32u + lane);
+                        r[4 * u] = __float_as_uint(t.x); r[4 * u + 1] = __float_as_uint(t.y);
+                        r[4 * u + 2] = __float_as_uint(t.z); r[4 * u + 3] = __float_as_uint(t.w);
+                    }
+                    tmem_st16(tb + (uint32_t)c, r);
+                }
+                tmem_st_wait();
+            }
+            tc_fence_before();
+            __syncwarp();
+            if (lane == 0) {
+                if (PAIR) mbar_arrive_cluster(smem_u32(&tmem_empty_bar[jn & 1]) & kPeerBitMask);
+                else mbar_arrive(smem_u32(&tmem_empty_bar[jn & 1]));
+            }
+        };
+        int cur = job_at(0);
+        if (SPLIT && cur >= 0) prep(0, cur);
+        for (int lt = 0; cur >= 0; ++lt) {
+            const int nxt = SPLIT ? job_at(lt + 1) : -1;
+            const bool defer = SPLIT && nxt >= 0 && is_source(cur) && has_pred(nxt);
+            if (SPLIT && nxt >= 0 && !defer) prep(lt + 1, nxt);
+            const int tile = cur & 0xFFFFFF;
             const int mt = (tile % m_work) * (PAIR ? 2 : 1) + (int)rank, rest = tile / m_work;
             const int ncol0 = (rest % p.n_blocks) * p.BN;
             const Phase& ph = p.phase[(rest / p.n_blocks) % p.nphase];
@@ -322,6 +500,23 @@
             mbar_wait(smem_u32(&tmem_full_bar[acc]), (uint32_t)((lt >> 1) & 1));
             tc_fence_after();
             const uint32_t trow = tmem_base + (uint32_t)(acc * kAccCols) + ((uint32_t)(q * 32) << 16);
+            if (is_source(cur)) {
+                const int j = tile - p.tail_base;
+                float4* dst = part_ws(j);
+                for (int c = 0; c < p.BN; c += 16) {
+                    uint32_t r[16];
+                    tmem_ld16(trow + (uint32_t)c, r);
+                    tmem_ld_wait();
+#pragma unroll
+                    for (int u = 0; u < 4; ++u)
+                        __stcg(dst + (size_t)(c / 4 + u) * 32u + lane,
+                               make_float4(__uint_as_float(r[4 * u]), __uint_as_float(r[4 * u + 1]), __uint_as_float(r[4 * u + 2]),
+                                           __uint_as_float(r[4 * u + 3])));
+                }
+                __threadfence();
+                __syncwarp();
+                if (lane == 0) st_release_gpu(part_flag(j), (unsigned int)(((cur >> 27) & 3) + 1));
+            } else
             if (p.tma_out) {
                 const int CH = p.out_f32 ? 32 : 64;
                 const int chs = p.out_f32 ? 5 : 6;
@@ -415,14 +610,7 @@
                         bulk_commit_group();
                     }
                 }
-                tc_fence_before();
-                __syncwarp();
-                if (lane == 0) {
-                    if (PAIR) mbar_arrive_cluster(smem_u32(&tmem_empty_bar[acc]) & kPeerBitMask);
-                    else mbar_arrive(smem_u32(&tmem_empty_bar[acc]));
-                }
-                continue;
-            }
+            } else {
             const int nchunks = p.BN >> 4;
             for (int ch = grp; ch < nchunks; ch += ngrp) {
                 uint32_t r[16];
@@ -473,11 +661,18 @@
                     }
                 }
             }
-            tc_fence_before();
-            __syncwarp();
-            if (lane == 0) {
-                if (PAIR) mbar_arrive_cluster(smem_u32(&tmem_empty_bar[acc]) & kPeerBitMask);
-                else mbar_arrive(smem_u32(&tmem_empty_bar[acc]));
+            }
+            if (SPLIT) {
+                if (defer) prep(lt + 1, nxt);
+                cur = nxt;
+            } else {
+                tc_fence_before();
+                __syncwarp();
+                if (lane == 0) {
+                    if (PAIR) mbar_arrive_cluster(smem_u32(&tmem_empty_bar[acc]) & kPeerBitMask);
+                    else mbar_arrive(smem_u32(&tmem_empty_bar[acc]));
+                }
+                cur = job_at(lt + 1);
             }
         }
     }
@@ -492,6 +687,16 @@
         if (warp == 0) tmem_dealloc<2 * kAccCols>(tmem_base);
     }
     if (p.sched != nullptr && rank == 0 && threadIdx.x == 0) sched_finish(p.sched, nworkers);
+    if (SPLIT && rank == 0 && threadIdx.x == 0) {
+        __threadfence();
+        if (atomicAdd(p.tail_ctl + kTailDoneOff, 1u) == (unsigned)(nworkers - 1)) {
+            const int L = total_tiles - p.tail_base;
+            for (int i = 0; i < 4 * L; ++i) p.tail_ctl[i] = 0u;
+            for (int i = 0; i < 8 * L; ++i) p.tail_ctl[kTailFlagOff + i] = 0u;
+            p.tail_ctl[kTailDoneOff] = 0u;
+            __threadfence();
+        }
+    }
 }
 
 template <bool PAIR>
@@ -930,6 +1135,56 @@
     return 0;
 }
 
+constexpr size_t kTailWsBytes = 20u << 20;
+static unsigned int* g_tail_ctl[64];
+static float* g_tail_ws[64];
+static int tail_scratch(unsigned int** ctl, float** ws, cudaStream_t st) {
+    const int dev = current_device();
+    SNN_REQUIRE(dev >= 0 && dev < 64, "bad CUDA device %d", dev);
+    *ctl = nullptr; *ws = nullptr;
+    static std::atomic<int> ready[64];
+    if (!ready[dev].load(std::memory_order_acquire)) {
+        cudaStreamCaptureStatus cs = cudaStreamCaptureStatusNone;
+        if (cudaStreamIsCapturing(st, &cs) != cudaSuccess || cs != cudaStreamCaptureStatusNone) return 0;
+        static PerDeviceOnce once;
+        SNN_CUDA_OK(once.run([dev] {
+            cudaError_t e = cudaMalloc(&g_tail_ctl[dev], sizeof(unsigned int) * kTailCtlWords);
+            if (e == cudaSuccess) e = cudaMemset(g_tail_ctl[dev], 0, sizeof(unsigned int) * kTailCtlWords);
+            if (e == cudaSuccess) e = cudaMalloc(&g_tail_ws[dev], kTailWsBytes);
+            if (e == cudaSuccess) e = cudaDeviceSynchronize();
+            return e;
+        }));
+        ready[dev].store(1, std::memory_order_release);
+    }
+    *ctl = g_tail_ctl[dev]; *ws = g_tail_ws[dev];
+    return 0;
+}
+
+constexpr double kTailMinPartFlop = 0.45e9;
+static int plan_tail(const ConvGemmParams& p, int total, int nw, bool small_k, bool pair) {
+    if (g_debug_flags[15] == 1 || p.sched != nullptr || p.ksplit > 1 || small_k || p.epi_groups != 1) return 0;
+    const bool force = g_debug_flags[15] >= 2;
+    int smin = 1 << 30;
+    for (int ph = 0; ph < p.nphase; ++ph) {
+        int S = 0;
+        for (int i = 0; i < p.phase[ph].nseg; ++i) S += (p.phase[ph].seg[i].nchunk + p.cps - 1) / p.cps;
+        smin = S < smin ? S : smin;
+    }
+    int kchunks = 0;
+    for (int i = 0; i < p.phase[0].nseg; ++i) kchunks += p.phase[0].seg[i].nchunk * p.ntap;
+    const double tile_flop = 2.0 * (pair ? 256 : 128) * p.BN * 64.0 * kchunks;
+    for (int q = 2; q <= 4; ++q) {
+        int base;
+        const int L = tail_split_tiles(total, nw, q, &base);
+        if (L == 0) continue;
+        if (smin < 2 * q || L > kTailMax) return 0;
+        if ((size_t)L * (pair ? 2 : 1) * 128 * p.BN * 4 > kTailWsBytes) return 0;
+        if (!force && tile_flop / q < kTailMinPartFlop * (q == 2 ? 1 : 4)) return 0;
+        return q;
+    }
+    return 0;
+}
+
 static int make_w_map(CUtensorMap* m, const void* ptr, int wN, int wT, int wK, int box_n);
 struct WDesc { const void* ptr; int wN, wT, wK; };
 
@@ -955,8 +1210,10 @@
     static PerDeviceOnce once;
     if (!t_plan.active) {
         SNN_CUDA_OK(once.run([] {
-            cudaError_t e = cudaFuncSetAttribute(conv_gemm_kernel<false>, cudaFuncAttributeMaxDynamicSharedMemorySize, 226 * 1024);
-            if (e == cudaSuccess) e = cudaFuncSetAttribute(conv_gemm_kernel<true>, cudaFuncAttributeMaxDynamicSharedMemorySize, 226 * 1024);
+            cudaError_t e = cudaFuncSetAttribute(conv_gemm_kernel<false, false>, cudaFuncAttributeMaxDynamicSharedMemorySize, 226 * 1024);
+            if (e == cudaSuccess) e = cudaFuncSetAttribute(conv_gemm_kernel<true, false>, cudaFuncAttributeMaxDynamicSharedMemorySize, 226 * 1024);
+            if (e == cudaSuccess) e = cudaFuncSetAttribute(conv_gemm_kernel<false, true>, cudaFuncAttributeMaxDynamicSharedMemorySize, 226 * 1024);
+            if (e == cudaSuccess) e = cudaFuncSetAttribute(conv_gemm_kernel<true, true>, cudaFuncAttributeMaxDynamicSharedMemorySize, 226 * 1024);
             return e;
         }));
     }
@@ -1006,14 +1263,26 @@
 #else
     p.dbg = 0;
 #endif
+    const int tiles = (pair ? (m_tiles + 1) / 2 : m_tiles) * p.n_blocks * p.nphase * p.ksplit;
+    int workers = pair ? num_sms() / 2 : num_sms();
+    if (g_debug_flags[5] > 0) workers = g_debug_flags[5];
+    if (workers > tiles) workers = tiles;
+    p.tail_q = plan_tail(p, tiles, workers, small_k, pair);
+    p.tail_base = tiles;
+    p.tail_absorb = g_debug_flags[15] == 3 ? 1 : 0;
+    int split_tiles = p.tail_q ? tail_split_tiles(tiles, workers, p.tail_q, &p.tail_base) : 0;
     if (t_plan.active) {
-        const int tiles = (pair ? (m_tiles + 1) / 2 : m_tiles) * p.n_blocks * p.nphase * p.ksplit;
-        const int workers = pair ? num_sms() / 2 : num_sms();
-        const int v[20] = {p.bn, p.bh, p.bw, p.BN, pair ? 1 : 0, p.ntap > 1 ? 1 : 0, p.hnw, p.stages, p.stage_bytes, p.cps, p.ksplit,
-                           tiles, p.n_blocks, workers < tiles ? workers : tiles, p.epi_groups, small_k ? 1 : 0, p.tma_out, (int)smem,
-                           p.a_bytes, p.b_bytes};
-        for (int i = 0; i < 20; ++i) t_plan.v[i] = v[i];
+        const int rounds = (tiles + workers - 1) / workers;
+        const int v[23] = {p.bn, p.bh, p.bw, p.BN, pair ? 1 : 0, p.ntap > 1 ? 1 : 0, p.hnw, p.stages, p.stage_bytes, p.cps, p.ksplit,
+                           tiles, p.n_blocks, workers, p.epi_groups, small_k ? 1 : 0, p.tma_out, (int)smem,
+                           p.a_bytes, p.b_bytes, p.tail_q ? p.tail_q : 1, split_tiles,
+                           p.tail_q ? p.tail_q * rounds - 1 : rounds};
+        for (int i = 0; i < 23; ++i) t_plan.v[i] = v[i];
         return 0;
+    }
+    if (p.tail_q) {
+        if (tail_scratch(&p.tail_ctl, &p.tail_ws, st)) return 2;
+        if (p.tail_ctl == nullptr) { p.tail_q = 0; p.tail_base = tiles; split_tiles = 0; }
     }
     CUtensorMap b, o;
     if (make_w_map(&b, wd.ptr, wd.wN, wd.wT, wd.wK, p.b_mn ? 64 : bn_cta)) return 2;
@@ -1027,17 +1296,10 @@
         o = b;
     }
     if (!pair) {
-        const int total_tiles = m_tiles * p.n_blocks * p.nphase * p.ksplit;
-        int grid = num_sms();
-        if (g_debug_flags[5] > 0) grid = g_debug_flags[5];
-        if (grid > total_tiles) grid = total_tiles;
-        return check_cuda(launch_pdl(conv_gemm_kernel<false>, dim3(grid), dim3(64 + 128 * p.epi_groups), smem, st, a0, a1, b, o, p),
+        return check_cuda(launch_pdl(p.tail_q ? conv_gemm_kernel<false, true> : conv_gemm_kernel<false, false>, dim3(workers), dim3(64 + 128 * p.epi_groups), smem, st, a0, a1, b, o, p),
                           "conv_gemm_kernel launch");
     }
-    const int total_tiles = ((m_tiles + 1) / 2) * p.n_blocks * p.nphase * p.ksplit;
-    int pairs = num_sms() / 2;
-    if (g_debug_flags[5] > 0) pairs = g_debug_flags[5];
-    if (pairs > total_tiles) pairs = total_tiles;
+    const int pairs = workers;
     cudaLaunchConfig_t cfg;
     memset(&cfg, 0, sizeof(cfg));
     cfg.gridDim = dim3(2 * pairs, 1, 1);
@@ -1051,7 +1313,8 @@
     attr[1].val.programmaticStreamSerializationAllowed = 1;
     cfg.attrs = attr;
     cfg.numAttrs = pdl_enabled() ? 2 : 1;
-    return check_cuda(cudaLaunchKernelEx(&cfg, conv_gemm_kernel<true>, a0, a1, b, o, p), "conv_gemm_kernel<pair> launch");
+    return check_cuda(cudaLaunchKernelEx(&cfg, p.tail_q ? conv_gemm_kernel<true, true> : conv_gemm_kernel<true, false>, a0, a1, b, o, p),
+                      "conv_gemm_kernel<pair> launch");
 }
 
 static int pick_bn(int n_store) {
@@ -1330,6 +1593,7 @@
         const int v[20] = {p.bn, p.bh, p.bw, p.NT, pair ? 1 : 0, p.strip, p.hnw, p.stages, p.stage_bytes, 1, p.ksplit, items, p.n_ci_tiles, nw, 1, 0, 1,
                            (int)smem, p.strip ? p.x_box_bytes : 8192, 2 * 8192};
         for (int i = 0; i < 20; ++i) t_plan.v[i] = v[i];
+        t_plan.v[20] = 1; t_plan.v[21] = 0; t_plan.v[22] = (items + nw - 1) / nw;
         return 0;
     }
     if (!pair) {
@@ -1364,8 +1628,10 @@
     else
         rc = conv_wgrad(geom, NB, H, W, dummy, Cin, Cin, dummy, Cout, Cout, static_cast<float*>(dummy), Cin, 0, nullptr);
     t_plan.active = false;
-    if (rc == 0) for (int i = 0; i < 20; ++i) out[i] = t_plan.v[i];
+    if (rc == 0) for (int i = 0; i < 23; ++i) out[i] = t_plan.v[i];
     return rc;
 }
 
-}
+int conv_tail_job(int items, int workers, int q, int w, int i) { return tail_job(i, w, workers, items, q > 1 ? q : 0); }
+
+}
diff --git a/snn_object_detectionddp_b200/kernels.py b/snn_object_detectionddp_b200/kernels.py
--- a/snn_object_detectionddp_b200/kernels.py
+++ b/snn_object_detectionddp_b200/kernels.py
@@ -131,17 +131,30 @@
 
 
 PLAN_FIELDS = ("bn", "bh", "bw", "n_tile", "pair", "strip", "hnw", "stages", "stage_bytes", "chunks_per_stage", "ksplit", "items",
-               "n_blocks", "ctas", "epi_groups", "small_k", "tma_out", "smem_bytes", "a_bytes", "b_bytes")
+               "n_blocks", "ctas", "epi_groups", "small_k", "tma_out", "smem_bytes", "a_bytes", "b_bytes", "tail_parts", "split_tiles",
+               "makespan")
 
 
 def conv_plan(kind, geom, nb, h, w, cin, cout, out_f32=True, frames_per_step=0, accumulate=False):
     import ctypes
-    out = (ctypes.c_int * 20)()
+    out = (ctypes.c_int * len(PLAN_FIELDS))()
     rc = _lib.lib().snn_conv_plan({"fprop": 0, "dgrad": 1, "wgrad": 2}[kind], geom, nb, h, w, cin, cout, int(out_f32), frames_per_step,
                              int(accumulate), out)
     if rc:
         raise _lib.SnnKernelError(f"snn_conv_plan failed (rc={rc}): {_lib.lib().snn_last_error().decode()}")
     return dict(zip(PLAN_FIELDS, list(out)))
+
+
+def tail_jobs(items, workers, tail_parts):
+    lib = _lib.lib()
+    jobs = []
+    for w in range(workers):
+        mine, i = [], 0
+        while (v := lib.snn_conv_tail_job(items, workers, tail_parts, w, i)) >= 0:
+            mine.append((v & 0xFFFFFF, v >> 24))
+            i += 1
+        jobs.append(mine)
+    return jobs
 
 
 def weight_prep(w_master, want_fprop=True, want_dgrad=True, wf=None, wt=None):
```
